# seulbinHwang/DiffusionDrive

Measured on AMD Instinct MI355X. Metric: scenes/s at batch 64, 2 denoise steps, 1/2/4/8 MI355X; waypoint L2 vs ref, higher is better.
Workload: dtype fp32 via f16x3 (each fp32 operand = hi+lo fp16, products ah*bh+ah*bl+al*bh, fp32 accumulate)

## Files before the change

diffusiondrive_amd/_lib.py:

```python
import ctypes
import os
import threading

HERE = os.path.dirname(os.path.abspath(__file__))
LIB_PATH = os.environ.get("DDMI_LIB", os.path.join(HERE, "libddmi.so"))

c_float_p = ctypes.POINTER(ctypes.c_float)
c_void_p = ctypes.c_void_p


class DDMIUnavailable(RuntimeError):
    """Raised when the native HIP library cannot be loaded."""


class DDMIError(RuntimeError):
    """Raised when a ddmi C-ABI call returns a non-zero status."""


class DDConfig(ctypes.Structure):
    _fields_ = [
        ("abi_version", ctypes.c_int), ("image_arch", ctypes.c_int), ("lidar_arch", ctypes.c_int),
        ("cam_h", ctypes.c_int), ("cam_w", ctypes.c_int), ("lidar_h", ctypes.c_int),
        ("lidar_w", ctypes.c_int), ("lidar_channels", ctypes.c_int), ("num_modes", ctypes.c_int),
        ("num_poses", ctypes.c_int), ("trunc_timestep", ctypes.c_int), ("step_span", ctypes.c_int),
    ]


class DDOutputs(ctypes.Structure):
    _fields_ = [
        ("trajectory", c_void_p), ("poses_reg", c_void_p), ("poses_cls", c_void_p),
        ("bev_semantic_map", c_void_p), ("agent_states", c_void_p), ("agent_labels", c_void_p),
    ]


class DDTrainOutputs(ctypes.Structure):
    _fields_ = [
        ("trajectory", c_void_p), ("poses_reg", c_void_p * 2), ("poses_cls", c_void_p * 2), ("loss", c_void_p),
        ("bev_semantic_map", c_void_p), ("agent_states", c_void_p), ("agent_labels", c_void_p),
    ]


class DDSampleOutputs(ctypes.Structure):
    _fields_ = [
        ("trajectory", c_void_p), ("poses_reg", c_void_p), ("poses_cls", c_void_p),
        ("best_trajectory", c_void_p), ("best_index", c_void_p),
        ("bev_semantic_map", c_void_p), ("agent_states", c_void_p), ("agent_labels", c_void_p),
    ]


class DDInputs(ctypes.Structure):
    _fields_ = [
        ("camera_f32", c_void_p), ("camera_u8", c_void_p), ("lidar_f32", c_void_p), ("lidar_u8", c_void_p),
        ("lidar_hist_max", ctypes.c_int), ("status", c_void_p), ("noise", c_void_p),
    ]


class DDSimParams(ctypes.Structure):
    _fields_ = [
        ("wheel_base", ctypes.c_double), ("dt", ctypes.c_double), ("tracking_horizon", ctypes.c_int),
        ("q_lon", ctypes.c_double), ("r_lon", ctypes.c_double), ("q_lat", ctypes.c_double * 3),
        ("r_lat", ctypes.c_double), ("jerk_penalty", ctypes.c_double), ("curvature_rate_penalty", ctypes.c_double),
        ("initial_curvature_penalty", ctypes.c_double), ("stopping_gain", ctypes.c_double),
        ("stopping_velocity", ctypes.c_double), ("max_steering_angle", ctypes.c_double),
        ("accel_time_constant", ctypes.c_double), ("steering_time_constant", ctypes.c_double),
    ]


class DDComfortParams(ctypes.Structure):
    _fields_ = [
        ("dt", ctypes.c_double), ("min_lon_accel", ctypes.c_double), ("max_lon_accel", ctypes.c_double),
        ("max_abs_lat_accel", ctypes.c_double), ("max_abs_mag_jerk", ctypes.c_double),
        ("max_abs_lon_jerk", ctypes.c_double), ("max_abs_yaw_accel", ctypes.c_double),
        ("max_abs_yaw_rate", ctypes.c_double),
    ]


class DDAreaParams(ctypes.Structure):
    _fields_ = [
        ("half_length", ctypes.c_double), ("half_width", ctypes.c_double), ("rear_axle_to_center", ctypes.c_double),
        ("dt", ctypes.c_double), ("driving_direction_horizon", ctypes.c_double),
        ("driving_direction_compliance_threshold", ctypes.c_double),
        ("driving_direction_violation_threshold", ctypes.c_double),
    ]


class DDDrivableMaps(ctypes.Structure):
    _fields_ = [
        ("verts", c_void_p), ("ring_off", c_void_p), ("poly_ring_off", c_void_p), ("poly_kind", c_void_p),
        ("scene_poly_off", c_void_p), ("num_polys", ctypes.c_int),
    ]


class DDOpView(ctypes.Structure):
    _fields_ = [("p", c_void_p), ("sn", ctypes.c_int64), ("sh", ctypes.c_int64), ("sw", ctypes.c_int64),
                ("sc", ctypes.c_int64)]


class DDOpConvDesc(ctypes.Structure):
    _fields_ = [
        ("in_", DDOpView), ("out", DDOpView), ("res", DDOpView),
        ("N", ctypes.c_int), ("H", ctypes.c_int), ("W", ctypes.c_int), ("Cin", ctypes.c_int),
        ("KH", ctypes.c_int), ("KW", ctypes.c_int), ("stride", ctypes.c_int), ("pad", ctypes.c_int),
        ("Cout", ctypes.c_int),
        ("wgt", c_void_p), ("ldb", ctypes.c_int64), ("k0", ctypes.c_int), ("bias", c_void_p),
        ("relu", ctypes.c_int), ("mode", ctypes.c_int), ("flags", c_void_p), ("route_rows", ctypes.c_int64),
        ("ln_out", c_void_p), ("ln_g", c_void_p), ("ln_b", c_void_p),
        ("pool_out", DDOpView), ("pool_p", ctypes.c_int), ("pool_add", DDOpView),
        ("fused_ln", ctypes.c_int), ("fused_pool", ctypes.c_int),
    ]


MAX_SAMPLES = 32

_SIGS = {
    "dd_default_config": (None, [ctypes.POINTER(DDConfig)]),
    "dd_create": (ctypes.c_int, [ctypes.POINTER(DDConfig), c_void_p, ctypes.c_size_t, ctypes.c_int,
                                 ctypes.POINTER(c_void_p)]),
    "dd_forward": (ctypes.c_int, [c_void_p, c_void_p, c_void_p, c_void_p, c_void_p, ctypes.c_int, ctypes.c_int,
                                  c_void_p, c_void_p, c_void_p, c_void_p]),
    "dd_forward_ex": (ctypes.c_int, [c_void_p, c_void_p, c_void_p, c_void_p, c_void_p, ctypes.c_int,
                                     ctypes.c_int, ctypes.POINTER(DDOutputs), c_void_p]),
    "dd_forward_samples": (ctypes.c_int, [c_void_p, c_void_p, c_void_p, c_void_p, c_void_p, ctypes.c_int,
                                          ctypes.c_int, ctypes.c_int, ctypes.POINTER(DDSampleOutputs), c_void_p]),
    "dd_forward_in": (ctypes.c_int, [c_void_p, ctypes.POINTER(DDInputs), ctypes.c_int, ctypes.c_int,
                                     ctypes.POINTER(DDOutputs), c_void_p]),
    "dd_forward_samples_in": (ctypes.c_int, [c_void_p, ctypes.POINTER(DDInputs), ctypes.c_int, ctypes.c_int,
                                             ctypes.c_int, ctypes.POINTER(DDSampleOutputs), c_void_p]),
    "dd_forward_train_in": (ctypes.c_int, [c_void_p, ctypes.POINTER(DDInputs), c_void_p, c_void_p, ctypes.c_int,
                                           ctypes.c_float, ctypes.c_float, c_void_p, c_void_p]),
    "dd_destroy": (ctypes.c_int, [c_void_p]),
    "dd_last_error": (ctypes.c_char_p, []),
    "dd_set_profiling": (ctypes.c_int, [c_void_p, ctypes.c_int]),
    "dd_reset_stats": (ctypes.c_int, [c_void_p]),
    "dd_kernel_stats": (ctypes.c_int, [c_void_p, ctypes.c_char_p, ctypes.POINTER(ctypes.c_double),
                                       ctypes.POINTER(ctypes.c_longlong), ctypes.POINTER(ctypes.c_double)]),
    "dd_kernel_bytes": (ctypes.c_int, [c_void_p, ctypes.c_char_p, ctypes.POINTER(ctypes.c_double)]),
    "dd_set_seed": (ctypes.c_int, [c_void_p, ctypes.c_ulonglong]),
    "dd_set_seed_at": (ctypes.c_int, [c_void_p, ctypes.c_ulonglong, ctypes.c_ulonglong]),
    "dd_set_graph": (ctypes.c_int, [c_void_p, ctypes.c_int]),
    "dd_set_streams": (ctypes.c_int, [c_void_p, ctypes.c_int]),
    "dd_get_streams": (ctypes.c_int, [c_void_p, ctypes.POINTER(ctypes.c_int)]),
    "dd_graph_info": (ctypes.c_int, [c_void_p, ctypes.POINTER(ctypes.c_int), ctypes.POINTER(ctypes.c_int),
                                     ctypes.POINTER(ctypes.c_int)]),
    "dd_graph_nodes": (ctypes.c_int, [c_void_p, ctypes.POINTER(ctypes.c_int), ctypes.POINTER(ctypes.c_int)]),
    "dd_forward_train": (ctypes.c_int, [c_void_p, c_void_p, c_void_p, c_void_p, c_void_p, c_void_p, c_void_p,
                                        ctypes.c_int, ctypes.c_float, ctypes.c_float, c_void_p, c_void_p]),
    "dd_bev_semantic_loss": (ctypes.c_int, [c_void_p, c_void_p, ctypes.c_int, ctypes.c_int, ctypes.c_int, ctypes.c_int,
                                            c_void_p, c_void_p, c_void_p]),
    "dd_bev_semantic_loss_work": (ctypes.c_size_t, [ctypes.c_int, ctypes.c_int, ctypes.c_int]),
    "dd_default_sim_params": (None, [ctypes.POINTER(DDSimParams)]),
    "dd_simulate_work": (ctypes.c_size_t, [ctypes.c_int]),
    "dd_simulate_proposals": (ctypes.c_int, [c_void_p, c_void_p, ctypes.c_int, ctypes.c_int,
                                             ctypes.POINTER(DDSimParams), c_void_p, c_void_p, c_void_p]),
    "dd_simulate": (ctypes.c_int, [c_void_p, ctypes.c_int, c_void_p, ctypes.c_int, ctypes.c_int,
                                   ctypes.POINTER(DDSimParams), c_void_p, c_void_p, c_void_p]),
    "dd_default_comfort_params": (None, [ctypes.POINTER(DDComfortParams)]),
    "dd_comfort": (ctypes.c_int, [c_void_p, ctypes.c_int, ctypes.POINTER(DDComfortParams), c_void_p, c_void_p,
                                  c_void_p]),
    "dd_default_area_params": (None, [ctypes.POINTER(DDAreaParams)]),
    "dd_ego_areas_work": (ctypes.c_size_t, [ctypes.c_int]),
    "dd_ego_areas": (ctypes.c_int, [c_void_p, ctypes.c_int, ctypes.c_int, ctypes.POINTER(DDDrivableMaps), ctypes.c_int,
                                    ctypes.POINTER(DDAreaParams), c_void_p, c_void_p, c_void_p, c_void_p, c_void_p,
                                    c_void_p]),
    "dd_set_gemm_mode": (ctypes.c_int, [c_void_p, ctypes.c_int]),
    "dd_set_schedule": (ctypes.c_int, [c_void_p, ctypes.c_int]),
    "dd_get_gemm_mode": (ctypes.c_int, [c_void_p, ctypes.POINTER(ctypes.c_int)]),
    "dd_numerics_flags": (ctypes.c_int, [c_void_p, ctypes.POINTER(ctypes.c_uint), ctypes.c_int]),
    "dd_tap": (ctypes.c_int, [c_void_p, ctypes.c_char_p, c_void_p, ctypes.c_size_t,
                              ctypes.POINTER(ctypes.c_size_t), c_void_p]),
    "dd_op_last_error": (ctypes.c_char_p, []),
    "dd_op_last_kernel": (ctypes.c_char_p, []),
    "dd_op_split_weights": (ctypes.c_int, [c_void_p, ctypes.c_int, ctypes.c_int, c_void_p, c_void_p, c_void_p, c_void_p,
                                           ctypes.POINTER(ctypes.c_int)]),
    "dd_op_pack_mk_weights": (ctypes.c_int, [c_void_p, ctypes.c_int, ctypes.c_int, c_void_p, c_void_p]),
    "dd_op_mk_linear": (ctypes.c_int, [c_void_p, ctypes.c_int, c_void_p, c_void_p, c_void_p, ctypes.c_int, c_void_p]),
    "dd_op_bevproj": (ctypes.c_int, [c_void_p, ctypes.c_int64, c_void_p, c_void_p, c_void_p, c_void_p, c_void_p, c_void_p,
                                     ctypes.c_int, ctypes.c_int, ctypes.c_int, ctypes.c_int, ctypes.c_int, c_void_p]),
    "dd_build_camera": (ctypes.c_int, [c_void_p, ctypes.c_int, ctypes.c_int, ctypes.c_int, c_void_p, ctypes.c_int,
                                       ctypes.c_int, c_void_p]),
    "dd_build_lidar": (ctypes.c_int, [c_void_p, c_void_p, ctypes.c_int, ctypes.c_int, c_void_p, ctypes.c_int,
                                      ctypes.c_float, ctypes.c_float, ctypes.c_int, ctypes.c_float, ctypes.c_float,
                                      ctypes.c_int, ctypes.c_longlong, c_void_p]),
    "dd_build_camera_u8": (ctypes.c_int, [c_void_p, ctypes.c_int, ctypes.c_int, ctypes.c_int, c_void_p, ctypes.c_int,
                                          ctypes.c_int, c_void_p]),
    "dd_build_lidar_u8": (ctypes.c_int, [c_void_p, c_void_p, ctypes.c_int, ctypes.c_int, c_void_p, ctypes.c_int,
                                         ctypes.c_float, ctypes.c_float, ctypes.c_int, ctypes.c_float, ctypes.c_float,
                                         ctypes.c_int, ctypes.c_longlong, c_void_p]),
    "dd_op_stem_pool_u8": (ctypes.c_int, [c_void_p, ctypes.c_int, ctypes.c_int, ctypes.c_int, ctypes.c_int,
                                          ctypes.c_int, c_void_p, c_void_p, c_void_p, c_void_p, ctypes.c_int, c_void_p,
                                          c_void_p]),
    "dd_op_conv2d": (ctypes.c_int, [c_void_p, ctypes.c_int, ctypes.c_int, ctypes.c_int, ctypes.c_int, c_void_p,
                                    c_void_p, c_void_p, c_void_p, ctypes.c_int, ctypes.c_int, ctypes.c_int,
                                    ctypes.c_int, ctypes.c_int, ctypes.c_int, c_void_p]),
    "dd_op_conv2d_x3": (ctypes.c_int, [c_void_p, ctypes.c_int, ctypes.c_int, ctypes.c_int, ctypes.c_int, c_void_p,
                                       c_void_p, c_void_p, c_void_p, ctypes.c_int, ctypes.c_int, ctypes.c_int,
                                       ctypes.c_int, ctypes.c_int, ctypes.c_int, ctypes.c_int, c_void_p, c_void_p]),
    "dd_op_stem_pool_x3": (ctypes.c_int, [c_void_p, ctypes.c_int, ctypes.c_int, ctypes.c_int, c_void_p, c_void_p,
                                          c_void_p, c_void_p, c_void_p]),
    "dd_op_stem_pool": (ctypes.c_int, [c_void_p, ctypes.c_int, ctypes.c_int, ctypes.c_int, c_void_p, c_void_p,
                                       c_void_p, ctypes.c_int, c_void_p, c_void_p]),
    "dd_op_stem_pool_nchw": (ctypes.c_int, [c_void_p, ctypes.c_int, ctypes.c_int, ctypes.c_int, ctypes.c_int, c_void_p,
                                            c_void_p, c_void_p, ctypes.c_int, c_void_p, c_void_p]),
    "dd_op_gemm": (ctypes.c_int, [c_void_p, ctypes.c_int, ctypes.c_int, c_void_p, c_void_p, c_void_p, c_void_p,
                                  ctypes.c_int, ctypes.c_int, c_void_p]),
    "dd_op_gemm_batched": (ctypes.c_int, [c_void_p, c_void_p, c_void_p, ctypes.c_int, ctypes.c_int, ctypes.c_int,
                                          ctypes.c_int, ctypes.c_int, c_void_p]),
    "dd_op_layernorm": (ctypes.c_int, [c_void_p, c_void_p, ctypes.c_int, c_void_p, c_void_p, c_void_p, c_void_p,
                                       c_void_p, ctypes.c_int, ctypes.c_int, c_void_p]),
    "dd_op_softmax_rows": (ctypes.c_int, [c_void_p, ctypes.c_int, ctypes.c_int, ctypes.c_float, c_void_p]),
    "dd_op_bilinear": (ctypes.c_int, [c_void_p, ctypes.c_int, ctypes.c_int, ctypes.c_int, ctypes.c_int, c_void_p,
                                      ctypes.c_int, ctypes.c_int, c_void_p]),
    "dd_op_bilinear_add": (ctypes.c_int, [c_void_p, ctypes.c_int, ctypes.c_int, ctypes.c_int, ctypes.c_int, c_void_p,
                                          ctypes.c_int, ctypes.c_int, c_void_p]),
    "dd_op_maxpool3x3s2": (ctypes.c_int, [c_void_p, ctypes.c_int, ctypes.c_int, ctypes.c_int, ctypes.c_int,
                                          c_void_p, c_void_p]),
    "dd_op_avgpool": (ctypes.c_int, [c_void_p, ctypes.c_int, ctypes.c_int, ctypes.c_int, ctypes.c_int,
                                     ctypes.c_int, ctypes.c_int, c_void_p, c_void_p]),
    "dd_op_bev_sample_attn": (ctypes.c_int, [c_void_p, c_void_p, c_void_p, c_void_p, ctypes.c_int, ctypes.c_int,
                                             ctypes.c_int, ctypes.c_int, ctypes.c_int, ctypes.c_int, c_void_p]),
    "dd_op_mha_small": (ctypes.c_int, [c_void_p, c_void_p, c_void_p, c_void_p, ctypes.c_int, ctypes.c_int,
                                       ctypes.c_int, ctypes.c_int, ctypes.c_int, c_void_p]),
    "dd_op_gpt_attention": (ctypes.c_int, [c_void_p, c_void_p, ctypes.c_int, ctypes.c_int, ctypes.c_int,
                                           ctypes.c_int, ctypes.c_int, c_void_p]),
    "dd_op_gpt_attention_rows": (ctypes.c_int, [c_void_p, c_void_p, ctypes.c_int, ctypes.c_int, ctypes.c_int,
                                                ctypes.c_int, ctypes.c_int, ctypes.c_int, ctypes.c_int, ctypes.c_int,
                                                c_void_p]),
    "dd_op_layernorm_groups": (ctypes.c_int, [c_void_p, c_void_p, c_void_p, c_void_p, ctypes.c_int, ctypes.c_int,
                                              ctypes.c_longlong, ctypes.c_int, c_void_p]),
    "dd_op_conv_desc_size": (ctypes.c_size_t, []),
    "dd_op_conv_view": (ctypes.c_int, [ctypes.POINTER(DDOpConvDesc), c_void_p]),
    "dd_op_layernorm_ld": (ctypes.c_int, [c_void_p, ctypes.c_int64, c_void_p, ctypes.c_int64, ctypes.c_int, c_void_p,
                                          c_void_p, c_void_p, c_void_p, ctypes.c_int, ctypes.c_int64, c_void_p,
                                          ctypes.c_int64, ctypes.c_int, ctypes.c_int, c_void_p]),
    "dd_op_bilinear_view": (ctypes.c_int, [ctypes.POINTER(DDOpView), ctypes.c_int, ctypes.c_int, ctypes.c_int,
                                           ctypes.c_int, ctypes.POINTER(DDOpView), ctypes.c_int, ctypes.c_int,
                                           ctypes.c_int, c_void_p]),
}

EXPORTED = tuple(_SIGS)

_lib = None
_lock = threading.Lock()


def load(path: str = None):
    global _lib
    with _lock:
        if _lib is not None and path is None:
            return _lib
        p = path or LIB_PATH
        if not os.path.exists(p):
            raise DDMIUnavailable(
                f"ddmi native library not found at {p}; build it with `python -m diffusiondrive_amd.build`")
        try:
            lib = ctypes.CDLL(p, mode=ctypes.RTLD_GLOBAL)
        except OSError as e:
            raise DDMIUnavailable(f"cannot load {p}: {e}") from e
        for name, (res, args) in _SIGS.items():
            fn = getattr(lib, name)
            fn.restype = res
            fn.argtypes = args
        if path is None:
            _lib = lib
        return lib


def check(rc: int, lib=None, op: bool = False):
    if rc != 0:
        lib = lib or load()
        msg = (lib.dd_op_last_error() if op else lib.dd_last_error()) or b""
        raise DDMIError(f"ddmi call failed (rc={rc}): {msg.decode(errors='replace')}")
    return rc
```

diffusiondrive_amd/csrc/common.h:

```cpp
#pragma once
#include <hip/hip_runtime.h>
#include <atomic>
#include <cstdint>
#include <stdexcept>
#include <string>

#define DD_HIP_CHECK(expr)                                                              \
  do {                                                                                   \
    hipError_t _e = (expr);                                                              \
    if (_e != hipSuccess)                                                                \
      throw std::runtime_error(std::string("HIP error ") + hipGetErrorString(_e) +      \
                               " at " __FILE__ ":" + std::to_string(__LINE__) + ": " #expr); \
  } while (0)

struct dd_sim_params;
struct dd_comfort_params;
struct dd_area_params;
struct dd_drivable_maps;

namespace ddmi {

inline void set_max_lds_once(std::atomic<uint64_t>& mask, const void* kernel, int bytes) {
  int dev = 0;
  DD_HIP_CHECK(hipGetDevice(&dev));
  const uint64_t bit = uint64_t(1) << (dev & 63);
  if (mask.load(std::memory_order_acquire) & bit) return;
  DD_HIP_CHECK(hipFuncSetAttribute(kernel, hipFuncAttributeMaxDynamicSharedMemorySize, bytes));
  mask.fetch_or(bit, std::memory_order_acq_rel);
}

struct View4 {
  float* p = nullptr;
  int64_t sn = 0, sh = 0, sw = 0, sc = 1;
};
inline View4 hwc(const float* p, int64_t sn, int W, int C) {
  return {const_cast<float*>(p), sn, (int64_t)W * C, C, 1};
}
inline View4 nhwc(const float* p, int H, int W, int C) { return hwc(p, (int64_t)H * W * C, W, C); }
inline View4 channels_from(View4 v, int64_t c0) {
  v.p += c0 * v.sc;
  return v;
}
inline View4 row_view(const float* p, int64_t gs, int64_t rs) { return {const_cast<float*>(p), gs, rs, 0, 1}; }

struct ConvArgs {
  const float* in = nullptr;
  int64_t in_sn = 0, in_sh = 0, in_sw = 0;
  int H = 1, W = 1, Cin = 0;
  const float* wgt = nullptr;
  int64_t ldb = 0;
  int b_kn = 0;
  const float* bias = nullptr;
  const float* res = nullptr;
  int64_t res_sn = 0, res_sh = 0, res_sw = 0;
  float* out = nullptr;
  int64_t out_sn = 0, out_sh = 0, out_sw = 0;
  int Nimg = 1, Ho = 1, Wo = 1, Cout = 0;
  int KH = 1, KW = 1, stride = 1, pad = 0;
  int relu = 0;
  float alpha = 1.0f;
  float* split_part = nullptr;
  int64_t split_cap = 0;
  int batch = 1, zdiv = 1;
  int64_t in_z1 = 0, in_z2 = 0, w_z1 = 0, w_z2 = 0, out_z1 = 0, out_z2 = 0, res_z1 = 0, res_z2 = 0;
  int64_t flops_K = -1;
  const uint16_t* wh = nullptr;
  const uint16_t* wl = nullptr;
  const float* wsinv = nullptr;
  int64_t ldh = 0;
  unsigned* flags = nullptr;
  int prec = 0;
  const int* rowmap = nullptr;
  int rowmap_nimg = 0;
  int rowmap_groups = 0;
  const int* rowcount = nullptr;
  int rowcap = 0;
  float* pool_out = nullptr;
  int pool_p = 0;
  int64_t pool_sn = 0, pool_sh = 0, pool_sw = 0;
  const float* pool_add = nullptr;
  int64_t pool_add_sh = 0, pool_add_sw = 0;
  float* ln_out = nullptr;
  const float* ln_g = nullptr;
  const float* ln_b = nullptr;
  int64_t route_rows = 0;
};
struct ConvGeom {
  int KH = 1, KW = 1, stride = 1, pad = 0, Cout = 0;
};
inline ConvArgs conv_args(View4 in, int N, int H, int W, int Cin, ConvGeom g, View4 out, int relu = 0,
                          View4 res = {}) {
  ConvArgs a;
  a.in = in.p;
  a.in_sn = in.sn;
  a.in_sh = in.sh;
  a.in_sw = in.sw;
  a.H = H;
  a.W = W;
  a.Cin = Cin;
  a.ldb = (int64_t)g.KH * g.KW * Cin;
  a.res = res.p;
  a.res_sn = res.sn;
  a.res_sh = res.sh;
  a.res_sw = res.sw;
  a.out = out.p;
  a.out_sn = out.sn;
  a.out_sh = out.sh;
  a.out_sw = out.sw;
  a.Nimg = N;
  a.Ho = (H + 2 * g.pad - g.KH) / g.stride + 1;
  a.Wo = (W + 2 * g.pad - g.KW) / g.stride + 1;
  a.Cout = g.Cout;
  a.KH = g.KH;
  a.KW = g.KW;
  a.stride = g.stride;
  a.pad = g.pad;
  a.relu = relu;
  return a;
}
inline ConvArgs gemm_args(View4 A, int G, int R, int K, int N, View4 C, int relu = 0, View4 res = {}) {
  return conv_args(A, G, R, 1, K, ConvGeom{1, 1, 1, 0, N}, C, relu, res);
}
inline void slice_k(ConvArgs& a, int k0, int64_t ldb) {
  a.wgt += k0;
  a.ldb = ldb;
  if (a.wh) a.wh += k0;
  if (a.wl) a.wl += k0;
}
inline void fold_ln(ConvArgs& a, float* y, const float* g, const float* b) {
  a.ln_out = y;
  a.ln_g = g;
  a.ln_b = b;
}
inline void pool_into(ConvArgs& a, int p, View4 out, View4 add) {
  a.pool_out = out.p;
  a.pool_p = p;
  a.pool_sn = out.sn;
  a.pool_sh = out.sh;
  a.pool_sw = out.sw;
  a.pool_add = add.p;
  a.pool_add_sh = add.sh;
  a.pool_add_sw = add.sw;
}
inline ConvArgs gathered_rows(ConvArgs a, const int* rowmap, int MR, int groups = 0, const int* counts = nullptr) {
  a.rowmap = rowmap;
  a.rowmap_nimg = a.Nimg;
  a.rowmap_groups = groups;
  if (counts) {
    a.rowcount = counts;
    a.rowcap = MR / groups;
  }
  a.Nimg = 1;
  a.Ho = MR;
  a.Wo = 1;
  return a;
}
constexpr unsigned DD_NUM_F16_OVERFLOW = 1u;
constexpr unsigned DD_NUM_SYNC_TIMEOUT = 2u;
constexpr unsigned DD_NUM_SYNC_STATE = 4u;
constexpr int kSplitMaxExp = 126;

#ifdef __HIPCC__
template <int BM, int NT>
__device__ inline void epi_row_table(const ConvArgs& a, int m0, int M, int tid, long long* tab,
                                     const int* rowidx = nullptr) {
  for (int r = tid; r < BM; r += NT) {
    const int m = rowidx ? rowidx[r] : m0 + r;
    long long oo = -1, ro = 0;
    if (m >= 0 && m < M) {
      const int ow = m % a.Wo, t2 = m / a.Wo;
      const int oh = t2 % a.Ho, n = t2 / a.Ho;
      oo = (long long)n * a.out_sn + (long long)oh * a.out_sh + (long long)ow * a.out_sw;
      ro = (long long)n * a.res_sn + (long long)oh * a.res_sh + (long long)ow * a.res_sw;
    }
    tab[2 * r] = oo;
    tab[2 * r + 1] = ro;
  }
}

__device__ inline void rowcount_prefix(const int* counts, int n, int* pre) {
  const int tid = threadIdx.x;
  if (tid < 64) {
    int c[4], s = 0;
#pragma unroll
    for (int j = 0; j < 4; ++j) {
      const int i = 4 * tid + j;
      c[j] = i < n ? counts[i] : 0;
      s += c[j];
    }
    int inc = s;
#pragma unroll
    for (int o = 1; o < 64; o <<= 1) {
      const int v = __shfl_up(inc, o, 64);
      if (tid >= o) inc += v;
    }
    int run = inc - s;
#pragma unroll
    for (int j = 0; j < 4; ++j) {
      const int i = 4 * tid + j;
      if (i <= n) pre[i] = run;
      run += c[j];
    }
    if (tid == 63 && n == 256) pre[256] = run;
  }
  __syncthreads();
}

__host__ __device__ inline bool epi_quads_ok(const ConvArgs& a) {
  auto al = [](const void* p) { return (reinterpret_cast<uintptr_t>(p) & 15) == 0; };
  auto st4 = [](int64_t s, int n) { return n == 1 || s % 4 == 0; };
  return a.Cout % 4 == 0 && al(a.out) && al(a.wsinv) && (!a.bias || al(a.bias)) && st4(a.out_sn, a.Nimg) &&
         st4(a.out_sh, a.Ho) && st4(a.out_sw, a.Wo) &&
         (!a.res || (al(a.res) && st4(a.res_sn, a.Nimg) && st4(a.res_sh, a.Ho) && st4(a.res_sw, a.Wo)));
}
template <int WM, int WN, int TM, int TN>
constexpr int epi_quads_lds() {
  return WM * 32 * WN * TN * 32 * 4 + WM * TM * 32 * 16;
}

template <int WM, int WN, int TM, int TN, typename Acc>
__device__ inline bool epi_quads(const ConvArgs& a, const Acc (&acc)[TM][TN], char* lds, int m0, int n0, int M,
                                 int tid, const int* rowidx = nullptr) {
  typedef float f4_t __attribute__((ext_vector_type(4)));
  constexpr int NT = 64 * WM * WN, BN = WN * TN * 32, QN = BN / 4, PR = WM * 32;
  constexpr int RPP = NT / QN, IT = PR / RPP;
  static_assert(NT % QN == 0 && PR % RPP == 0 && BN >= 64, "quad epilogue tiling");
  const int wave = tid >> 6, lane = tid & 63;
  const int wm = wave / WN, wn = wave % WN, li = lane & 31, hh = lane >> 5;
  float* ct = reinterpret_cast<float*>(lds);
  long long* tab = reinterpret_cast<long long*>(lds + PR * BN * 4);
  epi_row_table<WM * TM * 32, NT>(a, m0, M, tid, tab, rowidx);
  const int qn = tid % QN, nq = n0 + 4 * qn;
  const bool nv = nq < a.Cout;
  f4_t scl = {0.f, 0.f, 0.f, 0.f}, bia = {0.f, 0.f, 0.f, 0.f};
  if (nv) {
    scl = *reinterpret_cast<const f4_t*>(a.wsinv + nq) * a.alpha;
    if (a.bias) bia = *reinterpret_cast<const f4_t*>(a.bias + nq);
  }
  const bool ln = a.ln_out && BN == a.Cout && (QN == 16 || QN == 32 || QN == 64);
  f4_t lg = {0.f, 0.f, 0.f, 0.f}, lb = {0.f, 0.f, 0.f, 0.f};
  if (ln) {
    lg = *reinterpret_cast<const f4_t*>(a.ln_g + nq);
    lb = *reinterpret_cast<const f4_t*>(a.ln_b + nq);
  }
  bool bad = false;
#pragma unroll
  for (int i = 0; i < TM; ++i) {
    if (i) __syncthreads();
#pragma unroll
    for (int j = 0; j < TN; ++j)
#pragma unroll
      for (int r = 0; r < 16; ++r) {
        const int pr = wm * 32 + (r & 3) + 8 * (r >> 2) + 4 * hh;
        const int col = (wn * TN + j) * 32 + li;
        ct[pr * BN + ((((col >> 2) ^ (((pr >> 2) & 1) << 3))) << 2) + (col & 3)] = acc[i][j][r];
      }
    __syncthreads();
    f4_t rv[IT];
    long long oo[IT];
#pragma unroll
    for (int k = 0; k < IT; ++k) {
      const int pr = tid / QN + k * RPP;
      const int tr = ((pr >> 5) * TM + i) * 32 + (pr & 31);
      oo[k] = nv ? tab[2 * tr] : -1;
      rv[k] = (a.res && oo[k] >= 0) ? *reinterpret_cast<const f4_t*>(a.res + tab[2 * tr + 1] + nq)
                                    : (f4_t){0.f, 0.f, 0.f, 0.f};
    }
#pragma unroll
    for (int k = 0; k < IT; ++k) {
      if (oo[k] < 0) continue;
      const int pr = tid / QN + k * RPP;
      const f4_t c = *reinterpret_cast<const f4_t*>(ct + pr * BN + ((qn ^ (((pr >> 2) & 1) << 3)) << 2));
      bad |= !(__builtin_isfinite(c.x) && __builtin_isfinite(c.y) && __builtin_isfinite(c.z) &&
               __builtin_isfinite(c.w));
      f4_t v = c * scl + bia + rv[k];
      if (a.relu) {
        v.x = fmaxf(v.x, 0.f);
        v.y = fmaxf(v.y, 0.f);
        v.z = fmaxf(v.z, 0.f);
        v.w = fmaxf(v.w, 0.f);
      }
      __builtin_nontemporal_store(v, reinterpret_cast<f4_t*>(a.out + oo[k] + nq));
      if (ln) {
#pragma clang fp contract(off)
        float s = 0.f;
        s += (v.x + v.y) + (v.z + v.w);
#pragma unroll
        for (int o = QN / 2; o > 0; o >>= 1) s += __shfl_xor(s, o, 64);
        const float mean = s / (float)BN;
        const float dx = v.x - mean, dy = v.y - mean, dz = v.z - mean, dw = v.w - mean;
        float q = 0.f;
        q += (dx * dx + dy * dy) + (dz * dz + dw * dw);
#pragma unroll
        for (int o = QN / 2; o > 0; o >>= 1) q += __shfl_xor(q, o, 64);
        const float rstd = rsqrtf(q / (float)BN + 1e-5f);
        f4_t o4;
        o4.x = (v.x - mean) * rstd * lg.x + lb.x;
        o4.y = (v.y - mean) * rstd * lg.y + lb.y;
        o4.z = (v.z - mean) * rstd * lg.z + lb.z;
        o4.w = (v.w - mean) * rstd * lg.w + lb.w;
        *reinterpret_cast<f4_t*>(a.ln_out + oo[k] + nq) = o4;
      }
    }
  }
  return bad;
}
#endif
struct ConvRoute {
  const char* kernel = nullptr;
  const char* config = "";
  bool pooled = false;
  bool ln = false;
};
ConvRoute launch_conv_gemm(const ConvArgs& a, hipStream_t st);
ConvRoute launch_conv_x3(const ConvArgs& a, hipStream_t st);
ConvRoute launch_stem_pool(const ConvArgs& a, float* pool_out, int Hp, int Wp, hipStream_t st,
                           const void* const* src = nullptr, int src_c = 0, int u8 = 0, const float* lut = nullptr);
void launch_set_ptrs(const void** tab, const void* a, const void* b, hipStream_t st);
void launch_lidar_lut(float* lut, int hist_max, hipStream_t st);

struct VprojArgs {
  const float* map = nullptr;
  const uint16_t* wh = nullptr;
  const uint16_t* wl = nullptr;
  const float* wsinv = nullptr;
  int ldh = 0;
  const float* bias = nullptr;
  const int* rows = nullptr;
  const int* counts = nullptr;
  int B = 0, cap = 0;
  int nimg = 0;
  float* part = nullptr;
  float* out = nullptr;
  unsigned* flags = nullptr;
  int union_stage = 1;
  int umax = 1 << 30;
  unsigned* fb = nullptr;
  int fb_only = 0;
  int usplit = 1;
  unsigned* ucnt = nullptr;
};
bool vproj_supported(int C, int Cout, int H, int W);
size_t vproj_tiles(int B, int cap);
void launch_vproj(const VprojArgs& a, hipStream_t st);

void launch_nchw_to_nhwc(const float* in, float* out, int B, int C, int H, int W, int Cp, hipStream_t st);
void launch_u8_to_nhwc4(const uint8_t* in, float* out, int B, int C, int H, int W, int hwc, const float* lut,
                        hipStream_t st);
void launch_maxpool3x3s2(const float* in, float* out, int B, int H, int W, int C, int Ho, int Wo,
                         hipStream_t st);
void launch_avgpool(const float* in, int B, int H, int W, int C, int oh, int ow, View4 out,
                    const float* add, hipStream_t st);
void launch_bilinear(View4 in, int B, int Hi, int Wi, int C, View4 out, int Ho, int Wo, float ratio_h,
                     float ratio_w, int accumulate, hipStream_t st);
void launch_layernorm(const float* x, int64_t ldx, const float* res, int64_t ldres, int res_div,
                      const float* g, const float* b, const float* film_scale, const float* film_shift,
                      float* y, int64_t ldy, int rows, int C, hipStream_t st, int film_div = 0,
                      int64_t film_ld = 0, int group_rows = 0, int64_t group_stride = 0);
void launch_gpt_attention(const float* qkv, int B, int T, int C, int heads, float* y, int prec, hipStream_t st,
                          int q_first = 0, int q_count = -1, int nw_force = 0);
struct GptTailW {
  const uint16_t* wh = nullptr;
  const uint16_t* wl = nullptr;
  const float* sinv = nullptr;
  const float* bias = nullptr;
  int ldh = 0;
  float alpha = 1.0f;
};
struct GptTailArgs {
  const float* y = nullptr;
  float* x = nullptr;
  float* hb = nullptr;
  int M = 0, C = 0;
  GptTailW proj, up, down;
  const float *ln2_g = nullptr, *ln2_b = nullptr, *lnn_g = nullptr, *lnn_b = nullptr;
  unsigned* flags = nullptr;
};
bool gpt_tail_supported(int C);
void launch_gpt_tail(const GptTailArgs& a, hipStream_t st);
void launch_softmax_rows(float* x, int64_t ld, int rows, int L, float scale, hipStream_t st);
void launch_broadcast_rows(const float* src, int nsrc, float* dst, int rows, int C, hipStream_t st);
void launch_activation(const float* x, float* y, int64_t n, int act, hipStream_t st);
void launch_normal_philox(float* out, int64_t n, uint64_t seed, uint64_t first, hipStream_t st);

void launch_camera_feature(const uint8_t* cams, int B, int H, int W, float* out, int oh, int ow, hipStream_t st);
void launch_lidar_feature(const float* xyz, const int64_t* offs, int B, int C, float* out, int nb, float lo,
                          float hi, int ppm, float max_h, float split_h, int hist_max, int64_t max_points,
                          hipStream_t st);
void launch_camera_feature_u8(const uint8_t* cams, int B, int H, int W, uint8_t* out, int oh, int ow, hipStream_t st);
void launch_lidar_feature_u8(const float* xyz, const int64_t* offs, int B, int C, uint8_t* out, int nb, float lo,
                             float hi, int ppm, float max_h, float split_h, int hist_max, int64_t max_points,
                             hipStream_t st);

void launch_ddim_init(const float* anchor, const float* noise, float* img, int B, int QP, float sa,
                      float s1a, hipStream_t st);
void decoder_init_constants();
void launch_traj_embed(const float* img, float* pts, float* emb, int rows, int P, hipStream_t st);
void launch_timestep_embed(float t, float* out, int dim, hipStream_t st);
void launch_bev_sample_attn(const float* logits, const float* pts, const float* value, float* out,
                            int B, int Q, int P, int Hv, int Wv, int C, float inv_max_x,
                            float inv_max_y, hipStream_t st, int samples = 1);
void launch_bev_tap_rows(const float* pts, int* rows, int B, int Q, int P, int Hv, int Wv, float inv_max_x,
                         float inv_max_y, hipStream_t st, int samples = 1);
bool launch_bev_tap_dedup(const float* pts, int* rows, int* slots, int B, int Q, int P, int Hv, int Wv,
                          float inv_max_x, float inv_max_y, hipStream_t st, int samples = 1);
void launch_bev_sample_attn_gathered(const float* logits, const float* pts, const float* vrows, const int* slots,
                                     float* out, int B, int Q, int P, int Hv, int Wv, int C, float inv_max_x,
                                     float inv_max_y, hipStream_t st);
void launch_mha_small(const float* q, int64_t ldq, const float* k, const float* v, int64_t ldkv,
                      float* out, int64_t ldo, int B, int Lq, int Lk, int nh, int hd,
                      int64_t q_bstride, int64_t kv_bstride, int64_t o_bstride, hipStream_t st, int kv_div = 1);
void launch_reg_finalize(const float* r, const float* pts, float* reg, float* pts_next, int rows, int P,
                         hipStream_t st);
void launch_ddim_step(const float* reg, float* img, int rows, int P, float a_t, float a_prev,
                      hipStream_t st);
void launch_select_mode(const float* cls, const float* reg, float* traj, int* idx, int B, int Q, int P,
                        hipStream_t st);
void launch_select_best(const float* cls, const float* reg, float* traj, int* idx, int B, int N, int P,
                        hipStream_t st);
void launch_agent_post(float* states, int rows, hipStream_t st);

void launch_train_coeffs(const int* t, const float* ac, float* sa, float* s1a, int B, int tmax, hipStream_t st);
void launch_train_noisy(const float* anchor, const float* noise, const float* sa, const float* s1a, float* img, int B,
                        int QP, hipStream_t st);
void launch_timestep_embed_rows(const int* t, float* out, int B, int dim, hipStream_t st);
void launch_traj_loss_scene(const float* reg, const float* cls, const float* target, const float* anchor, float* part,
                            int B, int Q, int P, hipStream_t st);
void launch_traj_loss_reduce(const float* part, float* out, int B, int Q, int P, float cls_w, float reg_w,
                             hipStream_t st);
void launch_add2(float* o, hipStream_t st);
size_t bev_ce_partials(int B, int HW);
void launch_bev_ce(const float* logits, const uint8_t* target, float* part, float* out, int B, int C, int HW,
                   hipStream_t st);

size_t simulate_work_doubles(int N);
void launch_simulate(const float* traj, const double* proposals, const double* ego_states, int N, int per_group,
                     const dd_sim_params& p, double* work, double* out_states, hipStream_t st);

void launch_comfort(const double* states, int N, const dd_comfort_params& p, uint8_t* out_flags, double* out_signals,
                    hipStream_t st);

size_t ego_areas_work_doubles(int P);
void launch_ego_areas(const double* states, int N, int per_group, const dd_drivable_maps& maps, int G,
                      const dd_area_params& p, int horizon, double* work, uint8_t* out_areas, double* out_scores,
                      double* out_progress, double* out_coords, hipStream_t st);

}
```

diffusiondrive_amd/csrc/conv_x6.hip:

```cpp
#include <type_traits>

#include "common.h"


namespace ddmi {

namespace {

typedef _Float16 x6h8 __attribute__((ext_vector_type(8)));
typedef _Float16 x6h2 __attribute__((ext_vector_type(2)));
typedef float x6f2 __attribute__((ext_vector_type(2)));
typedef float x6f4 __attribute__((ext_vector_type(4)));
typedef float x6f16 __attribute__((ext_vector_type(16)));
typedef int x6i4 __attribute__((ext_vector_type(4)));
typedef __bf16 x6b8 __attribute__((ext_vector_type(8)));
typedef __bf16 x6b2 __attribute__((ext_vector_type(2)));

constexpr uint32_t kOOB6 = 0x80000000u;

__device__ inline x6i4 rsrc6(const void* p) {
  const uint64_t a = reinterpret_cast<uint64_t>(p);
  x6i4 r;
  r.x = (int)(uint32_t)a;
  r.y = (int)((uint32_t)(a >> 32) & 0xffffu);
  r.z = (int)kOOB6;
  r.w = 0x00020000;
  r.x = __builtin_amdgcn_readfirstlane(r.x);
  r.y = __builtin_amdgcn_readfirstlane(r.y);
  return r;
}

__device__ inline void dma6(x6i4 rsrc, uint32_t lds_wave, uint32_t voff) {
  asm volatile("s_mov_b32 m0, %0\n\tbuffer_load_dwordx4 %1, %2, 0 offen lds" ::"s"(lds_wave), "v"(voff), "s"(rsrc)
               : "memory");
}

__device__ inline x6f4 vload6(x6i4 rsrc, uint32_t voff) {
  x6f4 v;
  asm volatile("buffer_load_dwordx4 %0, %1, %2, 0 offen" : "=v"(v) : "v"(voff), "s"(rsrc) : "memory");
  return v;
}

template <int N>
__device__ inline void step_barrier() {
  static_assert(N >= 0 && N < 64, "vmcnt");
#ifdef DDMI_X6_NOBAR
  asm volatile("s_waitcnt vmcnt(%0) lgkmcnt(0)" ::"n"(N) : "memory");
#else
  asm volatile("s_waitcnt vmcnt(%0) lgkmcnt(0)\n\ts_barrier" ::"n"(N) : "memory");
#endif
}

template <int N>
__device__ inline void wait_vm() {
  static_assert(N >= 0 && N < 64, "vmcnt");
  asm volatile("s_waitcnt vmcnt(%0)" ::"n"(N) : "memory");
}

__device__ inline void split4(const x6f4 v, uint2& hi, uint2& lo) {
  const x6h2 h01 = __builtin_convertvector((x6f2){v.x, v.y}, x6h2);
  const x6h2 h23 = __builtin_convertvector((x6f2){v.z, v.w}, x6h2);
  const x6f2 f01 = __builtin_convertvector(h01, x6f2);
  const x6f2 f23 = __builtin_convertvector(h23, x6f2);
  const x6h2 l01 = __builtin_convertvector((x6f2){v.x - f01.x, v.y - f01.y}, x6h2);
  const x6h2 l23 = __builtin_convertvector((x6f2){v.z - f23.x, v.w - f23.y}, x6h2);
  hi = make_uint2(__builtin_bit_cast(uint32_t, h01), __builtin_bit_cast(uint32_t, h23));
  lo = make_uint2(__builtin_bit_cast(uint32_t, l01), __builtin_bit_cast(uint32_t, l23));
}

__device__ inline uint2 to_bf16x4(const x6f4 v) {
  const x6b2 b01 = __builtin_convertvector((x6f2){v.x, v.y}, x6b2);
  const x6b2 b23 = __builtin_convertvector((x6f2){v.z, v.w}, x6b2);
  return make_uint2(__builtin_bit_cast(uint32_t, b01), __builtin_bit_cast(uint32_t, b23));
}

constexpr bool halo_in_window(int t, int D, int TA, bool first) {
  for (int j = 1; j <= D; ++j) {
    const int u = t - j;
    if (first && u < 0) return false;
    if (((u % 9) + 9) % 9 == TA) return true;
  }
  return false;
}

}

#ifdef DDMI_X6_STAMPS
__device__ unsigned long long g_x6_st[8192 * 4];
extern "C" int dd_x6_stamps_read(unsigned long long* h, int n) {
  void* d = nullptr;
  if (hipGetSymbolAddress(&d, HIP_SYMBOL(g_x6_st)) != hipSuccess) return -1;
  if (hipMemcpy(h, d, (size_t)n * 8, hipMemcpyDeviceToHost) != hipSuccess) return -1;
  return hipMemset(d, 0, (size_t)n * 8) == hipSuccess ? 0 : -1;
}
#define X6_STAMP(k) x6st[k] = __builtin_amdgcn_s_memtime()
#else
#define X6_STAMP(k)
#endif

template <int TH, int TW, int BN, int WM, int WN, int D, int NSLOT, int SH, int PREC>
__global__ __launch_bounds__(64 * WM * WN, SH >= 2 ? SH + 1 : (SH ? (WM * WN == 8 ? 4 : 2) : 1)) void conv_x6_kernel(ConvArgs a, int tiles_x, int tiles_y, int n_sp,
                                                               int ntn, int nchunks) {
  constexpr int NW = WM * WN, NT = 64 * NW;
  constexpr int BM = TH * TW;
  constexpr int TM = BM / WM / 32;
  constexpr int TN = BN / WN / 32;
  static_assert(TM >= 1 && TN >= 1 && TM * WM * 32 == BM && TN * WN * 32 == BN, "wave tiling");
  static_assert(NSLOT >= D + 1 && D >= 1 && D <= 8, "ring");
  constexpr int P = TW + 2;
  constexpr int HP = (TH + 2) * P;
  constexpr int ABYTES = HP * 128;
  constexpr int BIMG = BN * 64;
  constexpr int BSLOT = 2 * BIMG;
  constexpr int BQ = BN / 16;
  constexpr int BPS = 2 * BQ / NW;
  static_assert(BPS >= 1 && (2 * BQ) % NW == 0 && BQ % BPS == 0, "B DMA split over the waves");
  constexpr int CH = PREC ? 64 : 32;
  constexpr int QP = CH / 4;
  constexpr int ALD = (HP * QP + NT - 1) / NT;
  constexpr int TA = 1;
  constexpr int NHB = SH ? 1 : 2;
  constexpr int B_OFF = NHB * ABYTES;
  constexpr int LDS_MAIN = NHB * ABYTES + NSLOT * BSLOT, LDS_EPI = BM * BN * 4;
  __shared__ __attribute__((aligned(1024))) char lds[LDS_MAIN > LDS_EPI ? LDS_MAIN : LDS_EPI];
  const uint32_t lds_u32 = (uint32_t)(uintptr_t)((__attribute__((address_space(3))) char*)lds);

  const int tid = threadIdx.x;
  const int lane = tid & 63;
  const int wave = __builtin_amdgcn_readfirstlane(tid >> 6);
#ifdef DDMI_X6_STAMPS
  unsigned long long x6st[4];
#endif
  X6_STAMP(0);

  const int nblk = n_sp * ntn;
  int tile = blockIdx.x;
  if (nblk >= 16) {
    const int q = nblk / 8, r = nblk % 8, x = tile % 8;
    tile = (x < r ? x * (q + 1) : r * (q + 1) + (x - r) * q) + tile / 8;
  }
  const int nt_idx = tile / n_sp;
  const int sp = tile - nt_idx * n_sp;
  const int txi = sp % tiles_x;
  const int t2 = sp / tiles_x;
  const int tyi = t2 % tiles_y;
  const int nimg = t2 / tiles_y;
  const int oy0 = tyi * TH, ox0 = txi * TW;
  const int n0 = nt_idx * BN;
  const int Cin = a.Cin;

  const x6i4 rin = rsrc6(a.in);

  constexpr bool HKEEP = NW == 8 && ALD <= 12 && !SH;
  auto hofs_of = [&](int i) {
    const int e = tid + NT * i;
    const int px = e / QP, q = e % QP;
    const int hy = px / P, hx = px - (px / P) * P;
    const int iy = oy0 - 1 + hy, ix = ox0 - 1 + hx;
    const bool in = px < HP && (unsigned)iy < (unsigned)a.H && (unsigned)ix < (unsigned)a.W;
    return in ? (int)(nimg * a.in_sn + iy * a.in_sh + ix * a.in_sw) + 4 * q : -1;
  };
  auto hwad_of = [&](int i) {
    const int e = tid + NT * i;
    const int px = e / QP, q = e % QP;
    const int q7 = q & 7, half = q >> 3;
    const int hx = px - (px / P) * P;
    return px < HP ? (px * 128 + ((((q7 >> 1) ^ (hx >> 1)) & 7) << 4) + ((q7 & 1) << 3)) ^ (half << 6) : -1;
  };
  int hofs[HKEEP ? ALD : 1], hwad[HKEEP ? ALD : 1];
  if constexpr (HKEEP) {
#pragma unroll
    for (int i = 0; i < ALD; ++i) {
      hofs[i] = hofs_of(i);
      hwad[i] = hwad_of(i);
    }
  }
  x6f4 hr[ALD];
  auto halo_issue = [&](int c) {
    const bool cv = c < nchunks;
    const int co = c * CH;
#pragma unroll
    for (int i = 0; i < ALD; ++i) {
      const int ho = HKEEP ? hofs[HKEEP ? i : 0] : hofs_of(i);
      hr[i] = vload6(rin, (cv && ho >= 0) ? (uint32_t)(ho + co) * 4u : kOOB6);
    }
  };
  auto halo_tie = [&]() {
#pragma unroll
    for (int i = 0; i < ALD; ++i) asm volatile("" : "+v"(hr[i]));
  };
  auto halo_store = [&](int buf) {
    char* base = lds + buf * ABYTES;
#pragma unroll
    for (int i = 0; i < ALD; ++i) {
      const int hw = HKEEP ? hwad[HKEEP ? i : 0] : hwad_of(i);
      if (hw < 0) continue;
      if constexpr (PREC == 1) {
        *reinterpret_cast<uint2*>(base + hw) = to_bf16x4(hr[i]);
      } else {
        uint2 hi, lo;
        split4(hr[i], hi, lo);
        *reinterpret_cast<uint2*>(base + hw) = hi;
        *reinterpret_cast<uint2*>(base + (hw ^ 64)) = lo;
      }
    }
  };

  uint32_t boff[BPS];
  bool bok[BPS];
  int brow[BPS];
#pragma unroll
  for (int j = 0; j < BPS; ++j) {
    const int qi = wave * BPS + j;
    const int rb = (qi % BQ) * 16;
    const int c = rb + (lane >> 2);
    const int ls = (lane & 3) ^ ((c >> 2) & 3);
    const int n = n0 + c;
    bok[j] = n < a.Cout;
    boff[j] = (uint32_t)(n * (int)a.ldh + ls * 8) * 2u;
    brow[j] = rb;
  }
  const bool bimg_lo = (wave * BPS) / BQ == 1;
  const x6i4 rwb = rsrc6((bimg_lo && !PREC) ? (const void*)a.wl : (const void*)a.wh);
  const uint32_t kb_lo = (PREC && bimg_lo) ? 64u : 0u;
  auto b_issue = [&](int slot, int tap, int c) {
    const bool cv = c < nchunks;
    const uint32_t kb = (uint32_t)(tap * Cin + c * CH) * 2u + kb_lo;
#pragma unroll
    for (int j = 0; j < BPS; ++j) {
      const uint32_t dst = lds_u32 + B_OFF + slot * BSLOT + (bimg_lo ? BIMG : 0) + brow[j] * 64;
      dma6(rwb, __builtin_amdgcn_readfirstlane(dst), (cv && bok[j]) ? boff[j] + kb : kOOB6);
    }
  };

  const int wm = wave / WN, wn = wave % WN;
  const int li = lane & 31, hh = lane >> 5;
  int aad[TM][3];
#pragma unroll
  for (int i = 0; i < TM; ++i) {
    const int m = (wm * TM + i) * 32 + li;
    const int y = m / TW, x = m % TW;
#pragma unroll
    for (int kw = 0; kw < 3; ++kw) aad[i][kw] = (y * P + x + kw) * 128 + (((hh ^ ((x + kw) >> 1)) & 7) << 4);
  }
  int bad_[TN];
#pragma unroll
  for (int j = 0; j < TN; ++j) {
    const int c = (wn * TN + j) * 32 + li;
    bad_[j] = c * 64 + (((hh ^ (c >> 2)) & 3) << 4);
  }

  x6f16 acc[TM][TN];
#pragma unroll
  for (int i = 0; i < TM; ++i)
#pragma unroll
    for (int j = 0; j < TN; ++j)
#pragma unroll
      for (int r = 0; r < 16; ++r) acc[i][j][r] = 0.f;

  constexpr bool PIPE = !(SH && NW == 8);
  struct Frag {
    x6h8 ah[TM], al[TM], bh[TN], bl[TN];
  };
  Frag F0, F1;
  auto load_frag = [&](Frag& F, int slot, int c, auto TAP, auto S2) {
    constexpr int t = decltype(TAP)::value, s2 = decltype(S2)::value;
    constexpr int kh = t / 3, kw = t % 3;
    const char* abuf = lds + (SH ? 0 : (c & 1)) * ABYTES + kh * P * 128;
    const char* bbuf = lds + B_OFF + slot * BSLOT;
#pragma unroll
    for (int j = 0; j < TN; ++j) {
      const int o = bad_[j] ^ (32 * s2);
      F.bh[j] = *reinterpret_cast<const x6h8*>(bbuf + o);
      F.bl[j] = *reinterpret_cast<const x6h8*>(bbuf + BIMG + o);
    }
#pragma unroll
    for (int i = 0; i < TM; ++i) {
      const int o = aad[i][kw] ^ (32 * s2);
      F.ah[i] = *reinterpret_cast<const x6h8*>(abuf + o);
      F.al[i] = *reinterpret_cast<const x6h8*>(abuf + (o ^ 64));
    }
  };
  auto mfma_frag = [&](const Frag& F) {
    if constexpr (PREC == 1) {
#pragma unroll
      for (int i = 0; i < TM; ++i)
#pragma unroll
        for (int j = 0; j < TN; ++j)
          acc[i][j] = __builtin_amdgcn_mfma_f32_32x32x16_bf16(__builtin_bit_cast(x6b8, F.ah[i]),
                                                             __builtin_bit_cast(x6b8, F.bh[j]), acc[i][j], 0, 0, 0);
#pragma unroll
      for (int i = 0; i < TM; ++i)
#pragma unroll
        for (int j = 0; j < TN; ++j)
          acc[i][j] = __builtin_amdgcn_mfma_f32_32x32x16_bf16(__builtin_bit_cast(x6b8, F.al[i]),
                                                             __builtin_bit_cast(x6b8, F.bl[j]), acc[i][j], 0, 0, 0);
      return;
    }
#pragma unroll
    for (int i = 0; i < TM; ++i)
#pragma unroll
      for (int j = 0; j < TN; ++j)
        acc[i][j] = __builtin_amdgcn_mfma_f32_32x32x16_f16(F.al[i], F.bh[j], acc[i][j], 0, 0, 0);
#pragma unroll
    for (int i = 0; i < TM; ++i)
#pragma unroll
      for (int j = 0; j < TN; ++j)
        acc[i][j] = __builtin_amdgcn_mfma_f32_32x32x16_f16(F.ah[i], F.bl[j], acc[i][j], 0, 0, 0);
#pragma unroll
    for (int i = 0; i < TM; ++i)
#pragma unroll
      for (int j = 0; j < TN; ++j)
        acc[i][j] = __builtin_amdgcn_mfma_f32_32x32x16_f16(F.ah[i], F.bh[j], acc[i][j], 0, 0, 0);
  };

  int slot = 0;
  auto open_step = [&](int c, auto TAP, auto FIRST) {
    constexpr int t = decltype(TAP)::value;
    constexpr bool first = decltype(FIRST)::value;
    constexpr int N = (D - 1) * BPS + (halo_in_window(t, D, TA, first) ? ALD : 0);
    step_barrier<N>();
    constexpr int tn = (t + D) % 9;
    int ns = slot + D;
    if (ns >= NSLOT) ns -= NSLOT;
    b_issue(ns, tn, t + D >= 9 ? c + 1 : c);
    if constexpr (t == TA) halo_issue(c + 1);
  };

  halo_issue(0);
#pragma unroll
  for (int u = 0; u < D; ++u) b_issue(u % NSLOT, u, 0);
  wait_vm<D * BPS>();
  halo_tie();
  halo_store(0);
  open_step(0, std::integral_constant<int, 0>(), std::true_type());
  if constexpr (PIPE) load_frag(F0, 0, 0, std::integral_constant<int, 0>(), std::integral_constant<int, 0>());

  auto step = [&](int c, auto TAP, auto FIRST) {
    constexpr int t = decltype(TAP)::value;
    constexpr bool first = decltype(FIRST)::value;
    if constexpr (!PIPE) {
      load_frag(F0, slot, c, TAP, std::integral_constant<int, 0>());
      mfma_frag(F0);
      load_frag(F0, slot, c, TAP, std::integral_constant<int, 1>());
      mfma_frag(F0);
      if constexpr (t == 8) {
        wait_vm<(8 - TA) * BPS>();
        halo_tie();
        asm volatile("s_waitcnt lgkmcnt(0)\n\ts_barrier" ::: "memory");
        halo_store(0);
      }
      if (++slot == NSLOT) slot = 0;
      open_step(t == 8 ? c + 1 : c, std::integral_constant<int, (t + 1) % 9>(),
                std::integral_constant<bool, first && t != 8>());
      return;
    }
    load_frag(F1, slot, c, TAP, std::integral_constant<int, 1>());
    __builtin_amdgcn_sched_barrier(0);
    mfma_frag(F0);
    if constexpr (t == 8) {
      wait_vm<(8 - TA) * BPS>();
      halo_tie();
      if constexpr (SH) {
        asm volatile("s_waitcnt lgkmcnt(0)\n\ts_barrier" ::: "memory");
        halo_store(0);
      } else {
        halo_store((c + 1) & 1);
      }
    }
    constexpr int t1 = (t + 1) % 9;
    const int c1 = t == 8 ? c + 1 : c;
    if (++slot == NSLOT) slot = 0;
    open_step(c1, std::integral_constant<int, t1>(), std::integral_constant<bool, first && t != 8>());
    load_frag(F0, slot, c1, std::integral_constant<int, t1>(), std::integral_constant<int, 0>());
    __builtin_amdgcn_sched_barrier(0);
    mfma_frag(F1);
    __builtin_amdgcn_sched_barrier(0);
  };
  auto chunk = [&](int c, auto FIRST) {
    step(c, std::integral_constant<int, 0>(), FIRST);
    step(c, std::integral_constant<int, 1>(), FIRST);
    step(c, std::integral_constant<int, 2>(), FIRST);
    step(c, std::integral_constant<int, 3>(), FIRST);
    step(c, std::integral_constant<int, 4>(), FIRST);
    step(c, std::integral_constant<int, 5>(), FIRST);
    step(c, std::integral_constant<int, 6>(), FIRST);
    step(c, std::integral_constant<int, 7>(), FIRST);
    step(c, std::integral_constant<int, 8>(), FIRST);
  };
  X6_STAMP(1);
  chunk(0, std::true_type());
  for (int c = 1; c < nchunks; ++c) chunk(c, std::false_type());
  step_barrier<0>();
  X6_STAMP(2);

  constexpr int QN = BN / 4;
  static_assert(NT % QN == 0, "epilogue quads");
  const int qn = tid % QN;
  const int nq = n0 + 4 * qn;
  const bool nv = nq < a.Cout;
  float* out = a.out + (int64_t)nimg * a.out_sn + nq;
  const float* res = a.res ? a.res + (int64_t)nimg * a.res_sn + nq : nullptr;
  const int osh = (int)a.out_sh, osw = (int)a.out_sw;
  const int rsh = (int)a.res_sh, rsw = (int)a.res_sw;
  constexpr int IT = BM / (NT / QN);
  constexpr bool EARLY = IT <= (NW == 8 && !SH ? 16 : 8);
  x6f4 rv[IT];
  int ooff[IT];
  auto load_res = [&]() {
#pragma unroll
    for (int k = 0; k < IT; ++k) {
      const int p = tid / QN + k * (NT / QN);
      const int oy = oy0 + p / TW, ox = ox0 + p % TW;
      const bool ok = nv && oy < a.Ho && ox < a.Wo;
      ooff[k] = ok ? oy * osh + ox * osw : -1;
      rv[k] = (res && ok) ? *reinterpret_cast<const x6f4*>(res + (oy * rsh + ox * rsw)) : (x6f4){0.f, 0.f, 0.f, 0.f};
    }
  };
  if constexpr (EARLY) load_res();
  x6f4 scl = {0.f, 0.f, 0.f, 0.f}, bia = {0.f, 0.f, 0.f, 0.f};
  if (nv) {
    scl = *reinterpret_cast<const x6f4*>(a.wsinv + nq) * a.alpha;
    if (a.bias) bia = *reinterpret_cast<const x6f4*>(a.bias + nq);
  }
  float* ct = reinterpret_cast<float*>(lds);
#pragma unroll
  for (int i = 0; i < TM; ++i)
#pragma unroll
    for (int j = 0; j < TN; ++j)
#pragma unroll
      for (int r = 0; r < 16; ++r) {
        const int m = (wm * TM + i) * 32 + (r & 3) + 8 * (r >> 2) + 4 * hh;
        ct[m * BN + (wn * TN + j) * 32 + li] = acc[i][j][r];
      }
  __syncthreads();
  if constexpr (!EARLY) load_res();
  bool bad = false;
#pragma unroll
  for (int k = 0; k < IT; ++k) {
    if (ooff[k] < 0) continue;
    const int p = tid / QN + k * (NT / QN);
    const x6f4 acc_v = *reinterpret_cast<const x6f4*>(ct + p * BN + 4 * qn);
    bad |= !(__builtin_isfinite(acc_v.x) && __builtin_isfinite(acc_v.y) && __builtin_isfinite(acc_v.z) &&
             __builtin_isfinite(acc_v.w));
    x6f4 v = acc_v * scl + bia + rv[k];
    if (a.relu) {
      v.x = fmaxf(v.x, 0.f);
      v.y = fmaxf(v.y, 0.f);
      v.z = fmaxf(v.z, 0.f);
      v.w = fmaxf(v.w, 0.f);
    }
    __builtin_nontemporal_store(v, reinterpret_cast<x6f4*>(out + ooff[k]));
    if (a.pool_out) *reinterpret_cast<x6f4*>(ct + p * BN + 4 * qn) = v;
  }
  if (a.pool_out) {
    __syncthreads();
    const int P = a.pool_p, WX = TW / P, NWIN = (TH / P) * WX;
    const float inv = 1.0f / (float)(P * P);
    for (int w = tid; w < NWIN * QN; w += NT) {
      const int win = w / QN, q = w - win * QN;
      const int nc = n0 + 4 * q;
      if (nc >= a.Cout) continue;
      const int wy = win / WX, wx = win - wy * WX;
      x6f4 sum = {0.f, 0.f, 0.f, 0.f};
      for (int dy = 0; dy < P; ++dy)
        for (int dx = 0; dx < P; ++dx)
          sum += *reinterpret_cast<const x6f4*>(ct + ((wy * P + dy) * TW + wx * P + dx) * BN + 4 * q);
      x6f4 v = sum * inv;
      const int py = oy0 / P + wy, px = ox0 / P + wx;
      if (a.pool_add) v += *reinterpret_cast<const x6f4*>(a.pool_add + py * a.pool_add_sh + px * a.pool_add_sw + nc);
      *reinterpret_cast<x6f4*>(a.pool_out + nimg * a.pool_sn + py * a.pool_sh + px * a.pool_sw + nc) = v;
    }
  }
  if (bad && a.flags) atomicOr(a.flags, (unsigned)DD_NUM_F16_OVERFLOW);
#ifdef DDMI_X6_STAMPS
  __syncthreads();
  X6_STAMP(3);
  if (tid == 0 && blockIdx.x < 8192)
    for (int k = 0; k < 4; ++k) g_x6_st[blockIdx.x * 4 + k] = x6st[k];
#endif
}

template <int TH, int TW, int BN, int WM, int WN, int D, int NSLOT, int SH, int PREC>
static void launch_x6_one(const ConvArgs& a_in, hipStream_t st, ConvRoute& r) {
  ConvArgs a = a_in;
  auto al16 = [](const void* p) { return (reinterpret_cast<uintptr_t>(p) & 15) == 0; };
  const bool pool = a.pool_out && a.pool_p >= 1 && TH % a.pool_p == 0 && TW % a.pool_p == 0 && a.Ho % TH == 0 &&
                    a.Wo % TW == 0 && al16(a.pool_out) && a.pool_sn % 4 == 0 && a.pool_sh % 4 == 0 &&
                    a.pool_sw % 4 == 0 && (!a.pool_add || (al16(a.pool_add) && a.pool_add_sh % 4 == 0 &&
                                                           a.pool_add_sw % 4 == 0));
  if (!pool) a.pool_out = nullptr;
  r.pooled = pool;
  const int tiles_x = (a.Wo + TW - 1) / TW, tiles_y = (a.Ho + TH - 1) / TH;
  const int n_sp = a.Nimg * tiles_x * tiles_y;
  const int ntn = (a.Cout + BN - 1) / BN;
  static const std::string name = "conv_x6<" + std::to_string(TH) + "," + std::to_string(TW) + "," +
                                  std::to_string(BN) + "," + std::to_string(WM) + "," + std::to_string(WN) +
                                  (PREC ? ",bf16>" : ">");
  r.config = name.c_str();
  hipLaunchKernelGGL((conv_x6_kernel<TH, TW, BN, WM, WN, D, NSLOT, SH, PREC>), dim3(n_sp * ntn), dim3(64 * WM * WN), 0,
                     st, a, tiles_x, tiles_y, n_sp, ntn, a.Cin / (PREC ? 64 : 32));
  DD_HIP_CHECK(hipGetLastError());
}
template <int TH, int TW, int BN, int WM, int WN, int D, int NSLOT, int SH>
static void launch_x6_cfg(const ConvArgs& a, hipStream_t st, ConvRoute& r) {
  if constexpr (SH == 0) {
    if (a.prec == 1) {
      launch_x6_one<TH, TW, BN, WM, WN, D, NSLOT, SH, 1>(a, st, r);
      return;
    }
  } else {
    if (a.prec == 1) throw std::runtime_error("conv_x6: bf16 takes the 8-wave configurations");
  }
  launch_x6_one<TH, TW, BN, WM, WN, D, NSLOT, SH, 0>(a, st, r);
}

bool launch_conv_x6(const ConvArgs& a, hipStream_t st, ConvRoute& r) {
  if ((a.prec != 0 && a.prec != 1) || a.KH != 3 || a.KW != 3 || a.stride != 1 || a.pad != 1 ||
      a.Cin % (a.prec ? 64 : 32) != 0 || a.batch != 1 || a.b_kn)
    return false;
  if (a.Ho != a.H || a.Wo != a.W || a.Ho < 8) return false;
  auto al16 = [](const void* p) { return (reinterpret_cast<uintptr_t>(p) & 15) == 0; };
  if (a.Cout % 4 || a.out_sw % 4 || a.out_sh % 4 || a.out_sn % 4 || !al16(a.out) || !al16(a.wsinv) ||
      (a.bias && !al16(a.bias)))
    return false;
  if (a.res && (a.res_sw % 4 || a.res_sh % 4 || a.res_sn % 4 || !al16(a.res))) return false;
  if ((int64_t)a.Nimg * a.in_sn >= (int64_t(1) << 29) || (int64_t)a.Cout * a.ldh >= (int64_t(1) << 30)) return false;
  if (a.Ho == 8 && a.Wo == 8 && a.Cout % 128 == 0) {
    if ((int64_t)a.Nimg * (a.Cout / 128) < 128) return false;
    launch_x6_cfg<8, 8, 128, 2, 4, 3, 4, 0>(a, st, r);
    return true;
  }
  const bool wide = a.Ho < 16;
  if (wide && a.Wo < 32) return false;
  const int64_t n_sp = (int64_t)a.Nimg * (wide ? ((a.Ho + 7) / 8) * ((a.Wo + 31) / 32)
                                               : ((a.Ho + 15) / 16) * ((a.Wo + 15) / 16));
  const bool bn128 = a.Cout > 64 && n_sp * ((a.Cout + 127) / 128) >= 256;
  const bool sh4 = a.prec == 0 && a.Cin <= 64;
  const bool b128 = bn128;
#define X6(TH, TW, BN, WM, WN, D, NS, SH) launch_x6_cfg<TH, TW, BN, WM, WN, D, NS, SH>(a, st, r)
  {
    const int64_t wgs = b128 ? n_sp * ((a.Cout + 127) / 128) : n_sp * ((a.Cout + 63) / 64);
    const char* se = getenv("DDMI_X6_SMALL");
    const int sm = se ? atoi(se) : 1;
    if (sm == 2 || (wgs < 128 && sm != 0)) {
      X6(8, 8, 64, 2, 2, 2, 3, 0);
      return true;
    }
  }
  if (wide) {
    if (b128) {
      X6(8, 32, 128, 4, 2, 3, 4, 0);
    } else {
      if (sh4) X6(8, 32, 64, 4, 1, 2, 3, 1); else X6(8, 32, 64, 4, 2, 2, 3, 0);
    }
  } else {
    if (b128) {
      X6(16, 16, 128, 4, 2, 3, 4, 0);
    } else {
      if (sh4) X6(16, 16, 64, 4, 1, 2, 3, 1); else X6(16, 16, 64, 4, 2, 2, 3, 0);
    }
  }
#undef X6
  return true;
}

}
```

diffusiondrive_amd/csrc/ops_abi.cpp:

```cpp
#include <cmath>
#include <cstring>
#include <string>

#include "../../include/ddmi.h"
#include "common.h"
#include "decoder_mk.h"
#include "weights.h"
#include <vector>

namespace {
thread_local std::string g_op_err;
thread_local const char* g_op_kernel = "";
void ran(const ddmi::ConvRoute& r) {
  if (*r.config) g_op_kernel = r.config;
}

template <class F>
int op_guard(F&& f) {
  try {
    f();
    return DD_OK;
  } catch (const std::invalid_argument& e) {
    g_op_err = e.what();
    return DD_ERR_INVALID;
  } catch (const std::exception& e) {
    g_op_err = e.what();
    return DD_ERR_RUNTIME;
  }
}
hipStream_t S(void* s) { return static_cast<hipStream_t>(s); }
}

using namespace ddmi;

extern "C" {

const char* dd_op_last_error(void) { return g_op_err.c_str(); }

const char* dd_op_last_kernel(void) { return g_op_kernel; }

int dd_op_split_weights(const float* w, int rows, int K, uint16_t* hi, uint16_t* lo, uint16_t* b16, float* sinv,
                        int* ldh_out) {
  return op_guard([&] {
    if (!w || rows < 1 || K < 1) throw std::invalid_argument("dd_op_split_weights: null pointer or bad shape");
    Arena ar;
    const SplitW x = prep_split(ar, w, rows, K);
    const size_t bytes = (size_t)rows * x.ldh * sizeof(uint16_t);
    if (hi) std::memcpy(hi, ar.host(x.hi), bytes);
    if (lo) std::memcpy(lo, ar.host(x.lo), bytes);
    if (b16) std::memcpy(b16, ar.host(x.b16), bytes);
    if (sinv) std::memcpy(sinv, ar.host(x.sinv), (size_t)rows * sizeof(float));
    if (ldh_out) *ldh_out = x.ldh;
  });
}

int dd_op_pack_mk_weights(const float* w, int nout, int nin, uint16_t* packed, float* sinv) {
  return op_guard([&] {
    if (!w || nout < 1 || nin < 1 || nin % 16 || nout % 32)
      throw std::invalid_argument("dd_op_pack_mk_weights: null pointer, nin % 16 or nout % 32");
    std::vector<_Float16> pk;
    std::vector<float> si;
    pack_mk_weights(w, nout, nin, pk, si);
    if (packed) std::memcpy(packed, pk.data(), pk.size() * sizeof(_Float16));
    if (sinv) std::memcpy(sinv, si.data(), si.size() * sizeof(float));
  });
}

int dd_op_mk_linear(const float* A, int K, const float* wgt, const float* bias, float* out, int N, void* stream) {
  return op_guard([&] {
    std::vector<float> hw((size_t)N * K);
    DD_HIP_CHECK(hipStreamSynchronize(S(stream)));
    DD_HIP_CHECK(hipMemcpy(hw.data(), wgt, hw.size() * sizeof(float), hipMemcpyDeviceToHost));
    std::vector<_Float16> pk;
    std::vector<float> sinv;
    pack_mk_weights(hw.data(), N, K, pk, sinv);
    Arena ar;
    const size_t wo = ar.add(reinterpret_cast<const float*>(pk.data()), pk.size() / 2);
    const size_t so = ar.add(sinv);
    ar.upload();
    MkLin m;
    m.w = reinterpret_cast<const uint4*>(ar.ptr(wo));
    m.s = ar.ptr(so);
    m.b = bias;
    m.nks = K / 16;
    launch_mk_linear_test(A, K, m, N, out, S(stream));
    DD_HIP_CHECK(hipStreamSynchronize(S(stream)));
  });
}

int dd_op_bevproj(const float* p3, int64_t p3_ld, const float* kvp, const float* wgt, const float* bias,
                  const float* ln_g, const float* ln_b, float* out, int B, int H, int W, int Hk, int Wk, void* stream) {
  return op_guard([&] {
    if (!bevproj_supported(256, 64, H, W, Hk, Wk)) throw std::invalid_argument("dd_op_bevproj: unsupported shape");
    std::vector<float> hw((size_t)256 * 64);
    DD_HIP_CHECK(hipStreamSynchronize(S(stream)));
    DD_HIP_CHECK(hipMemcpy(hw.data(), wgt, hw.size() * sizeof(float), hipMemcpyDeviceToHost));
    std::vector<_Float16> pk;
    std::vector<float> sinv;
    pack_mk_weights(hw.data(), 256, 64, pk, sinv);
    Arena ar;
    const size_t wo = ar.add(reinterpret_cast<const float*>(pk.data()), pk.size() / 2);
    const size_t so = ar.add(sinv);
    ar.upload();
    BevProjArgs a;
    a.p3 = p3;
    a.p3_ld = p3_ld;
    a.kvp = kvp;
    a.w = reinterpret_cast<const uint4*>(ar.ptr(wo));
    a.s = ar.ptr(so);
    a.bias = bias;
    a.g = ln_g;
    a.beta = ln_b;
    a.out = out;
    a.B = B;
    a.H = H;
    a.W = W;
    a.Hk = Hk;
    a.Wk = Wk;
    launch_bevproj(a, S(stream));
    DD_HIP_CHECK(hipStreamSynchronize(S(stream)));
  });
}

static ConvArgs conv2d_args(const float* in, int B, int H, int W, int Cin, const float* wgt, const float* bias,
                            const float* res, float* out, int Cout, int KH, int KW, int stride, int pad, int relu) {
  const int Ho = (H + 2 * pad - KH) / stride + 1, Wo = (W + 2 * pad - KW) / stride + 1;
  ConvArgs a = conv_args(nhwc(in, H, W, Cin), B, H, W, Cin, ConvGeom{KH, KW, stride, pad, Cout},
                         nhwc(out, Ho, Wo, Cout), relu, nhwc(res, Ho, Wo, Cout));
  a.wgt = wgt;
  a.bias = bias;
  return a;
}
static void attach_split(ConvArgs& a, const Arena& ar, const SplitW& x, int prec, unsigned* flags) {
  a.prec = prec;
  a.wh = reinterpret_cast<const uint16_t*>(ar.ptr(prec ? x.b16 : x.hi));
  a.wl = reinterpret_cast<const uint16_t*>(ar.ptr(x.lo));
  a.wsinv = ar.ptr(x.sinv);
  a.ldh = x.ldh;
  a.flags = flags;
}

int dd_op_conv2d(const float* in, int B, int H, int W, int Cin, const float* wgt, const float* bias, const float* res,
                 float* out, int Cout, int KH, int KW, int stride, int pad, int relu, void* stream) {
  return op_guard([&] {
    ran(launch_conv_gemm(conv2d_args(in, B, H, W, Cin, wgt, bias, res, out, Cout, KH, KW, stride, pad, relu),
                         S(stream)));
  });
}

int dd_op_conv2d_x3(const float* in, int B, int H, int W, int Cin, const float* wgt, const float* bias,
                    const float* res, float* out, int Cout, int KH, int KW, int stride, int pad, int relu, int prec,
                    unsigned* flags, void* stream) {
  return op_guard([&] {
    const int K = KH * KW * Cin;
    std::vector<float> hw((size_t)Cout * K);
    DD_HIP_CHECK(hipStreamSynchronize(S(stream)));
    DD_HIP_CHECK(hipMemcpy(hw.data(), wgt, hw.size() * sizeof(float), hipMemcpyDeviceToHost));
    Arena ar;
    const SplitW x = prep_split(ar, hw.data(), Cout, K);
    ar.upload();
    ConvArgs a = conv2d_args(in, B, H, W, Cin, wgt, bias, res, out, Cout, KH, KW, stride, pad, relu);
    if (prec != 0 && prec != 1) throw std::invalid_argument("prec must be 0 (f16x3) or 1 (bf16)");
    attach_split(a, ar, x, prec, flags);
    const int64_t mo = (int64_t)B * a.Ho * a.Wo * Cout;
    float* part = nullptr;
    if (prec == 0 && mo <= (1 << 20)) {
      DD_HIP_CHECK(hipMalloc(&part, (size_t)(8 * mo) * sizeof(float)));
      a.split_part = part;
      a.split_cap = 8 * mo;
    }
    ran(launch_conv_gemm(a, S(stream)));
    const hipError_t e = hipStreamSynchronize(S(stream));
    if (part) DD_HIP_CHECK(hipFree(part));
    DD_HIP_CHECK(e);
  });
}

static int dd_op_stem_pool_impl(const void* in, int src_c, int B, int H, int W, const float* wgt, const float* bias,
                                float* out, int prec, unsigned* flags, void* stream, int u8 = 0,
                                const float* lut = nullptr);

int dd_op_stem_pool_u8(const uint8_t* in, int layout, int B, int C, int H, int W, const float* lut, const float* wgt,
                       const float* bias, float* out, int prec, unsigned* flags, void* stream) {
  if (!in || !lut || (layout != 0 && layout != 1) || C < 1 || C > 3 || (layout == 0 && C != 3))
    return op_guard([&] {
      throw std::invalid_argument("stem_pool_u8: layout 0 (HWC, C = 3) or 1 (planar, C = 1..3), in and lut non-null");
    });
  return dd_op_stem_pool_impl(in, C, B, H, W, wgt, bias, out, prec, flags, stream, layout == 0 ? 1 : 2, lut);
}

int dd_op_stem_pool_x3(const float* in, int B, int H, int W, const float* wgt, const float* bias, float* out,
                       unsigned* flags, void* stream) {
  return dd_op_stem_pool(in, B, H, W, wgt, bias, out, 0, flags, stream);
}

int dd_op_stem_pool_nchw(const float* in, int B, int C, int H, int W, const float* wgt, const float* bias, float* out,
                         int prec, unsigned* flags, void* stream) {
  if (C < 1 || C > 3) return op_guard([&] { throw std::invalid_argument("stem_pool_nchw: C must be 1..3"); });
  return dd_op_stem_pool_impl(in, C, B, H, W, wgt, bias, out, prec, flags, stream);
}

int dd_op_stem_pool(const float* in, int B, int H, int W, const float* wgt, const float* bias, float* out, int prec,
                    unsigned* flags, void* stream) {
  return dd_op_stem_pool_impl(in, 0, B, H, W, wgt, bias, out, prec, flags, stream);
}

static int dd_op_stem_pool_impl(const void* in, int src_c, int B, int H, int W, const float* wgt, const float* bias,
                                float* out, int prec, unsigned* flags, void* stream, int u8, const float* lut) {
  return op_guard([&] {
    if (prec != 0 && prec != 1) throw std::invalid_argument("stem_pool: prec must be 0 (f16x3) or 1 (bf16)");
    const int Cin = 4, Cout = 64, K = 7 * 7 * Cin;
    std::vector<float> hw((size_t)Cout * K);
    DD_HIP_CHECK(hipStreamSynchronize(S(stream)));
    DD_HIP_CHECK(hipMemcpy(hw.data(), wgt, hw.size() * sizeof(float), hipMemcpyDeviceToHost));
    Arena ar;
    const SplitW x = prep_split(ar, hw.data(), Cout, K);
    ar.upload();
    ConvArgs a = conv_args(nhwc(u8 ? nullptr : static_cast<const float*>(in), H, W, Cin), B, H, W, Cin,
                           ConvGeom{7, 7, 2, 3, Cout}, View4{}, true);
    a.wgt = wgt;
    a.bias = bias;
    attach_split(a, ar, x, prec, flags);
    const int hp = (a.Ho + 2 - 3) / 2 + 1, wp = (a.Wo + 2 - 3) / 2 + 1;
    const void** word = nullptr;
    if (src_c) {
      DD_HIP_CHECK(hipMalloc(reinterpret_cast<void**>(&word), sizeof(const void*)));
      DD_HIP_CHECK(hipMemcpy(word, &in, sizeof(const void*), hipMemcpyHostToDevice));
    }
    bool ok = false;
    try {
      const ConvRoute r = launch_stem_pool(a, out, hp, wp, S(stream), src_c ? word : nullptr, src_c, u8, lut);
      ran(r);
      ok = r.kernel != nullptr;
      DD_HIP_CHECK(hipStreamSynchronize(S(stream)));
    } catch (...) {
      if (word) (void)hipFree(word);
      throw;
    }
    if (word) DD_HIP_CHECK(hipFree(word));
    if (!ok) throw std::invalid_argument("stem_pool: shape not supported");
  });
}

int dd_build_camera(const uint8_t* cams, int B, int src_h, int src_w, float* out, int out_h, int out_w,
                    void* stream) {
  return op_guard([&] {
    if (!cams || !out) throw std::invalid_argument("null pointer");
    launch_camera_feature(cams, B, src_h, src_w, out, out_h, out_w, S(stream));
  });
}

int dd_build_lidar(const float* xyz, const int64_t* offsets, int B, int channels, float* out, int resolution,
                   float range_lo, float range_hi, int pixels_per_meter, float max_height, float split_height,
                   int hist_max, long long max_points, void* stream) {
  return op_guard([&] {
    if (!offsets || !out || (!xyz && max_points > 0)) throw std::invalid_argument("null pointer");
    launch_lidar_feature(xyz, offsets, B, channels, out, resolution, range_lo, range_hi, pixels_per_meter,
                         max_height, split_height, hist_max, max_points, S(stream));
  });
}

int dd_build_camera_u8(const uint8_t* cams, int B, int src_h, int src_w, uint8_t* out, int out_h, int out_w,
                       void* stream) {
  return op_guard([&] {
    if (!cams || !out) throw std::invalid_argument("null pointer");
    launch_camera_feature_u8(cams, B, src_h, src_w, out, out_h, out_w, S(stream));
  });
}

int dd_build_lidar_u8(const float* xyz, const int64_t* offsets, int B, int channels, uint8_t* out, int resolution,
                      float range_lo, float range_hi, int pixels_per_meter, float max_height, float split_height,
                      int hist_max, long long max_points, void* stream) {
  return op_guard([&] {
    if (!offsets || !out || (!xyz && max_points > 0)) throw std::invalid_argument("null pointer");
    launch_lidar_feature_u8(xyz, offsets, B, channels, out, resolution, range_lo, range_hi, pixels_per_meter,
                            max_height, split_height, hist_max, max_points, S(stream));
  });
}

int dd_op_gemm(const float* A, int M, int K, const float* W, const float* bias, const float* res, float* C, int N,
               int relu, void* stream) {
  return op_guard([&] {
    ConvArgs a = gemm_args(row_view(A, K, K), M, 1, K, N, row_view(C, N, N), relu, row_view(res, N, N));
    a.wgt = W;
    a.bias = bias;
    ran(launch_conv_gemm(a, S(stream)));
  });
}

int dd_op_gemm_batched(const float* A, const float* Bm, float* C, int batch, int M, int N, int K, int kn,
                       void* stream) {
  return op_guard([&] {
    ConvArgs a = gemm_args(row_view(A, K, K), M, 1, K, N, row_view(C, N, N));
    a.wgt = Bm;
    a.ldb = kn ? N : K;
    a.b_kn = kn;
    a.batch = batch;
    a.zdiv = 1;
    a.in_z1 = (int64_t)M * K;
    a.w_z1 = (int64_t)K * N;
    a.out_z1 = (int64_t)M * N;
    ran(launch_conv_gemm(a, S(stream)));
  });
}

int dd_op_layernorm(const float* x, const float* res, int res_div, const float* g, const float* b,
                    const float* film_scale, const float* film_shift, float* y, int rows, int C, void* stream) {
  return op_guard([&] {
    launch_layernorm(x, C, res, C, res_div, g, b, film_scale, film_shift, y, C, rows, C, S(stream));
  });
}

int dd_bev_semantic_loss(const float* logits, const unsigned char* target, int B, int C, int H, int W, float* work,
                         float* loss, void* stream) {
  return op_guard([&] {
    if (!logits || !target || !work || !loss || B < 1 || C < 1 || C > 255 || H < 1 || W < 1)
      throw std::invalid_argument("dd_bev_semantic_loss: null pointer or bad shape");
    launch_bev_ce(logits, target, work, loss, B, C, H * W, S(stream));
  });
}

size_t dd_bev_semantic_loss_work(int B, int H, int W) { return bev_ce_partials(B, H * W); }

int dd_op_softmax_rows(float* x, int rows, int L, float scale, void* stream) {
  return op_guard([&] { launch_softmax_rows(x, L, rows, L, scale, S(stream)); });
}

int dd_op_bilinear(const float* in, int B, int Hi, int Wi, int C, float* out, int Ho, int Wo, void* stream) {
  return op_guard([&] {
    View4 a{const_cast<float*>(in), (int64_t)Hi * Wi * C, (int64_t)Wi * C, C, 1};
    View4 o{out, (int64_t)Ho * Wo * C, (int64_t)Wo * C, C, 1};
    launch_bilinear(a, B, Hi, Wi, C, o, Ho, Wo, (float)Hi / (float)Ho, (float)Wi / (float)Wo, 0, S(stream));
  });
}

int dd_op_bilinear_add(const float* in, int B, int Hi, int Wi, int C, float* out, int Ho, int Wo, void* stream) {
  return op_guard([&] {
    View4 a{const_cast<float*>(in), (int64_t)Hi * Wi * C, (int64_t)Wi * C, C, 1};
    View4 o{out, (int64_t)Ho * Wo * C, (int64_t)Wo * C, C, 1};
    launch_bilinear(a, B, Hi, Wi, C, o, Ho, Wo, (float)Hi / (float)Ho, (float)Wi / (float)Wo, 1, S(stream));
  });
}

int dd_op_maxpool3x3s2(const float* in, int B, int H, int W, int C, float* out, void* stream) {
  return op_guard([&] {
    const int Ho = (H + 2 - 3) / 2 + 1, Wo = (W + 2 - 3) / 2 + 1;
    launch_maxpool3x3s2(in, out, B, H, W, C, Ho, Wo, S(stream));
  });
}

int dd_op_avgpool(const float* in, int B, int H, int W, int C, int oh, int ow, float* out, void* stream) {
  return op_guard([&] {
    View4 o{out, (int64_t)oh * ow * C, (int64_t)ow * C, C, 1};
    launch_avgpool(in, B, H, W, C, oh, ow, o, nullptr, S(stream));
  });
}

int dd_op_bev_sample_attn(const float* logits, const float* pts, const float* value, float* out, int B, int Q, int P,
                          int Hv, int Wv, int C, void* stream) {
  return op_guard([&] {
    launch_bev_sample_attn(logits, pts, value, out, B, Q, P, Hv, Wv, C, 1.0f / 32.0f, 1.0f / 32.0f, S(stream));
  });
}

int dd_op_mha_small(const float* q, const float* k, const float* v, float* out, int B, int Lq, int Lk, int nh, int hd,
                    void* stream) {
  return op_guard([&] {
    const int d = nh * hd;
    launch_mha_small(q, d, k, v, d, out, d, B, Lq, Lk, nh, hd, (int64_t)Lq * d, (int64_t)Lk * d, (int64_t)Lq * d,
                     S(stream));
  });
}

int dd_op_gpt_attention(const float* qkv, float* y, int B, int T, int C, int heads, int prec, void* stream) {
  return op_guard([&] { launch_gpt_attention(qkv, B, T, C, heads, y, prec, S(stream)); });
}

int dd_op_gpt_attention_rows(const float* qkv, float* y, int B, int T, int C, int heads, int prec, int q_first,
                             int q_count, int waves, void* stream) {
  return op_guard([&] {
    if (q_count < 1) throw std::invalid_argument("dd_op_gpt_attention_rows: q_count < 1");
    launch_gpt_attention(qkv, B, T, C, heads, y, prec, S(stream), q_first, q_count, waves);
  });
}

int dd_op_layernorm_groups(const float* x, const float* g, const float* b, float* y, int groups, int group_rows,
                           long long group_stride, int C, void* stream) {
  return op_guard([&] {
    if (groups < 1 || group_rows < 1 || group_stride < (long long)group_rows * C)
      throw std::invalid_argument("dd_op_layernorm_groups: groups, group_rows >= 1 and non-overlapping groups");
    launch_layernorm(x, C, nullptr, 0, 1, g, b, nullptr, nullptr, y, C, groups * group_rows, C, S(stream), 0, 0,
                     group_rows, group_stride);
  });
}

size_t dd_op_conv_desc_size(void) { return sizeof(dd_op_conv_desc); }

static View4 view_of(const dd_op_view& v) { return {v.p, v.sn, v.sh, v.sw, v.sc}; }

int dd_op_conv_view(dd_op_conv_desc* d, void* stream) {
  return op_guard([&] {
    if (!d) throw std::invalid_argument("dd_op_conv_view: null descriptor");
    d->fused_ln = d->fused_pool = 0;
    if (!d->in.p || !d->out.p || !d->wgt) throw std::invalid_argument("dd_op_conv_view: null in, out or wgt");
    if (d->mode < 0 || d->mode > 2) throw std::invalid_argument("dd_op_conv_view: mode must be 0, 1 or 2");
    if (d->N < 1 || d->H < 1 || d->W < 1 || d->Cin < 1 || d->Cout < 1 || d->KH < 1 || d->KW < 1 || d->stride < 1 ||
        d->pad < 0)
      throw std::invalid_argument("dd_op_conv_view: bad geometry");
    for (const dd_op_view* v : {&d->in, &d->out, &d->res, &d->pool_out, &d->pool_add})
      if (v->p && v->sc != 1) throw std::invalid_argument("dd_op_conv_view: the operands' channel stride is 1");
    const int64_t K = (int64_t)d->KH * d->KW * d->Cin;
    const bool sliced = d->k0 != 0 || d->ldb != K;
    if (sliced && (d->KH != 1 || d->KW != 1 || d->k0 < 0 || d->k0 % 8 || d->Cin % 8 || d->k0 + K > d->ldb))
      throw std::invalid_argument("dd_op_conv_view: a K slice needs a 1 x 1 geometry, k0 % 8 == 0, Cin % 8 == 0 and "
                                  "k0 + Cin <= ldb");
    const ConvGeom g{d->KH, d->KW, d->stride, d->pad, d->Cout};
    const bool rows = d->KH == 1 && d->KW == 1 && d->stride == 1 && d->pad == 0 && d->W == 1;
    ConvArgs a = rows ? gemm_args(view_of(d->in), d->N, d->H, d->Cin, d->Cout, view_of(d->out), d->relu,
                                  view_of(d->res))
                      : conv_args(view_of(d->in), d->N, d->H, d->W, d->Cin, g, view_of(d->out), d->relu,
                                  view_of(d->res));
    a.wgt = d->wgt;
    a.bias = d->bias;
    a.route_rows = d->route_rows;
    Arena ar;
    DD_HIP_CHECK(hipStreamSynchronize(S(stream)));
    if (d->mode) {
      std::vector<float> hw((size_t)d->Cout * d->ldb);
      DD_HIP_CHECK(hipMemcpy(hw.data(), d->wgt, hw.size() * sizeof(float), hipMemcpyDeviceToHost));
      const SplitW x = prep_split(ar, hw.data(), d->Cout, (int)d->ldb);
      ar.upload();
      attach_split(a, ar, x, d->mode - 1, d->flags);
    }
    if (sliced) slice_k(a, d->k0, d->ldb);
    if (d->ln_out) fold_ln(a, d->ln_out, d->ln_g, d->ln_b);
    if (d->pool_out.p) pool_into(a, d->pool_p, view_of(d->pool_out), view_of(d->pool_add));
    const int64_t mo = (int64_t)a.Nimg * a.Ho * a.Wo * a.Cout;
    float* part = nullptr;
    if (d->mode == 1 && mo <= (1 << 20)) {
      DD_HIP_CHECK(hipMalloc(&part, (size_t)(8 * mo) * sizeof(float)));
      a.split_part = part;
      a.split_cap = 8 * mo;
    }
    hipError_t e = hipSuccess;
    try {
      const ConvRoute r = launch_conv_gemm(a, S(stream));
      ran(r);
      d->fused_ln = r.ln;
      d->fused_pool = r.pooled;
      e = hipStreamSynchronize(S(stream));
    } catch (...) {
      if (part) (void)hipFree(part);
      throw;
    }
    if (part) DD_HIP_CHECK(hipFree(part));
    DD_HIP_CHECK(e);
  });
}

int dd_op_layernorm_ld(const float* x, int64_t ldx, const float* res, int64_t ldres, int res_div, const float* g,
                       const float* b, const float* film_scale, const float* film_shift, int film_div,
                       int64_t film_ld, float* y, int64_t ldy, int rows, int C, void* stream) {
  return op_guard([&] {
    if (!x || !y || !g || !b || rows < 0 || C < 1 || ldx < C || ldy < C)
      throw std::invalid_argument("dd_op_layernorm_ld: null pointer or a leading dimension below C");
    launch_layernorm(x, ldx, res, ldres, res_div, g, b, film_scale, film_shift, y, ldy, rows, C, S(stream), film_div,
                     film_ld);
  });
}

int dd_op_bilinear_view(const dd_op_view* in, int B, int Hi, int Wi, int C, const dd_op_view* out, int Ho, int Wo,
                        int accumulate, void* stream) {
  return op_guard([&] {
    if (!in || !out || !in->p || !out->p || B < 1 || Hi < 1 || Wi < 1 || C < 1 || Ho < 1 || Wo < 1)
      throw std::invalid_argument("dd_op_bilinear_view: null view or bad shape");
    launch_bilinear(view_of(*in), B, Hi, Wi, C, view_of(*out), Ho, Wo, (float)Hi / (float)Ho, (float)Wi / (float)Wo,
                    accumulate, S(stream));
  });
}

}
```

diffusiondrive_amd/csrc/runtime.cpp:

```cpp
#include <cmath>
#include <cstdio>
#include <cstdlib>
#include <cstring>
#include <map>
#include <memory>
#include <mutex>
#include <set>
#include <type_traits>
#include <vector>

#ifdef DDMI_SEGV_TRACE
#define DD_TRACE(...) (fprintf(stderr, "[ddmi-trace] " __VA_ARGS__), fputc('\n', stderr), fflush(stderr))
#else
#define DD_TRACE(...) ((void)0)
#endif
#include "../../include/ddmi.h"
#include "common.h"
#include "decoder_mk.h"
#include "weights.h"

namespace ddmi {

struct Block {
  bool bottleneck = false;
// ... 746 lines not shown
      ia.rows = rows_of(0, 0);
      ia.slots = slots_of(0, 0);
      ia.counts = counts_of(0, 0);
      ia.sa = vanilla ? 0.0f : std::sqrt(a8);
      ia.s1a = vanilla ? 1.0f : std::sqrt(1.0f - a8);
      if (c.train) {
        ia.sa_b = bufs.at("train_sa").first;
        ia.s1a_b = bufs.at("train_s1a").first;
      }
      ia.B = B;
      ia.samples = S;
      launch("decoder", 0, [&] { launch_decoder_mk_init(ia, st); });
      launch("misc", 0, [&] {
        launch_mk_prefetch(W(mk_w_begin), (mk_w_end - mk_w_begin) * sizeof(float), st);
      });
    }
    const MkLayer layers[2] = {mk_layer(0), mk_layer(1)};
    MkAnchor anc;
    anc.pa0 = mk(m_pa0);
    anc.pa3 = mk(m_pa3);
    anc.pa2g = W(pa2.g);
    anc.pa2b = W(pa2.b);
    float* reg_last = nullptr;
    float* cls_last = nullptr;
    for (int si = 0; si < steps; ++si) {
      for (int l = 0; l < 2; ++l) {
        const std::string sf = sfx(si, l);
        float* vrows = buf("value_rows" + sf, (size_t)MR * d);
        gathered_value(l, rows_of(si, l), counts_of(si, l), vrows, cross, B, B / S, HB, WB, MR,
                       tf_pending ? tf_scenes : 0);
        if (tf_pending) {
          join();
          tf_pending = false;
        }
        MkArgs m;
        m.L = layers[l];
        m.A = anc;
        m.layer = l;
        m.B = B;
        m.samples = S;
        m.imgx = imgx;
        m.tfe = tfe;
        m.pts = l == 0 ? pts : pts2;
        m.pts_next = l == 0 ? pts2 : nullptr;
        m.vrows = vrows;
        m.slots = slots_of(si, l);
        m.akv = akv[l];
        m.ego = egos[l];
        if (c.train) {
          m.film = bufs.at("train_film_l" + std::to_string(l)).first;
          m.film_stride = 2 * d;
        } else {
          m.film = buf("film_s" + std::to_string(si) + "l" + std::to_string(l), 2 * d);
        }
        m.gs_out = buf("gs" + sf, (size_t)R * d);
        m.reg_out = buf("reg" + sf, (size_t)R * P * 3);
        m.cls_out = buf("cls" + sf, R);
        if (l == 0) {
          m.next_rows = rows_of(si, 1);
          m.next_slots = slots_of(si, 1);
          m.next_counts = counts_of(si, 1);
        } else if (si + 1 < steps) {
          m.next_rows = rows_of(si + 1, 0);
          m.next_slots = slots_of(si + 1, 0);
          m.next_counts = counts_of(si + 1, 0);
          const int k = roll[si];
          const float a_t = ac[k], a_p = (k - ratio >= 0) ? ac[k - ratio] : 1.0f;
          m.ddim = 1;
          m.sa_t = std::sqrt(a_t);
          m.sb_t = std::sqrt(1.0f - a_t);
          m.sa_p = std::sqrt(a_p);
          m.sdir = std::sqrt(1.0f - a_p);
        } else {
          m.traj = traj;
          m.mode_idx = idx;
        }
        m.flags = num_flags;
        m.dim_t = W(dim_t_off);
        m.groups = mk_stamps ? 1 : (mk_groups_env ? mk_groups_env : (B * 4 <= 64 ? 4 : (B * 2 <= 64 ? 2 : 1)));
        if (m.groups > 1) {
          m.scene_cnt = reinterpret_cast<unsigned*>(buf_zeroed("mk_scene_cnt", (size_t)B));
          m.next_pts = buf("mk_next_pts", (size_t)R * P * 2);
          m.cls_x = buf("mk_cls_x", (size_t)B * 32);
        }
        if (mk_stamps) m.stamps = reinterpret_cast<unsigned long long*>(buf("mk_stamps" + sf, (size_t)B * 80));
        double kn = 7.0 * d * d + 2.0 * d * 1024 + (double)d * (P + 1 + 3 * P);
        if (l == 0) kn += 512.0 * d + (double)d * d;
        launch("decoder", 2.0 * R * kn, [&] { launch_decoder_mk(m, st); }, nullptr, -1.0, groups_note(m.groups));
        reg_last = m.reg_out;
        cls_last = m.cls_out;
      }
    }
    join();
    alias("poses_reg", reg_last);
    alias("poses_cls", cls_last);
    train_loss_partials(c, B);
  }

  const float* W(size_t off) const { return ar.ptr(off); }

  int num_cus() {
    if (!cu_count) {
      int dev = 0;
      DD_HIP_CHECK(hipGetDevice(&dev));
      DD_HIP_CHECK(hipDeviceGetAttribute(&cu_count, hipDeviceAttributeMultiprocessorCount, dev));
    }
    return cu_count;
  }
  int cu_count = 0;

  float* buf_zeroed(const std::string& name, size_t n) {
    const uint64_t g = generation;
    float* p = buf(name, n);
    if (generation != g) DD_HIP_CHECK(hipMemsetAsync(p, 0, std::max<size_t>(n, 4) * sizeof(float), st));
    return p;
  }

  float* buf(const std::string& name, size_t n) {
    auto it = bufs.find(name);
    if (it != bufs.end() && it->second.second >= n) return it->second.first;
    if (it != bufs.end()) {
      DD_HIP_CHECK(hipFree(it->second.first));
      bufs.erase(it);
    }
    float* p = nullptr;
    DD_HIP_CHECK(hipMalloc(&p, std::max<size_t>(n, 4) * sizeof(float)));
    bufs[name] = {p, n};
    ++generation;
    return p;
  }

  hipEvent_t fj_event() {
    if (fj_next == fj_ev.size()) {
      hipEvent_t e;
      DD_HIP_CHECK(hipEventCreateWithFlags(&e, hipEventDisableTiming));
      fj_ev.push_back(e);
    }
    return fj_ev[fj_next++];
  }
  bool sides() const { return use_side && !profiling; }

  bool seg_cap = false;
  int seg_s = 0;
  hipStream_t st_cap = nullptr;
  Program* seg_prog = nullptr;
  void seg_begin(int s) {
    seg_s = s;
    DD_HIP_CHECK(hipStreamBeginCapture(st_cap, hipStreamCaptureModeThreadLocal));
  }
  void seg_end() {
    hipGraph_t g = nullptr;
    DD_HIP_CHECK(hipStreamEndCapture(st_cap, &g));
    size_t n = 0, roots = 0;
    hipError_t e = hipGraphGetNodes(g, nullptr, &n);
    if (e == hipSuccess) e = hipGraphGetRootNodes(g, nullptr, &roots);
    if (e == hipSuccess && n > 0) {
      if (roots > 1) ++seg_prog->branched;
      std::vector<hipGraphNode_t> nodes(n);
      e = hipGraphGetNodes(g, nodes.data(), &n);
      for (size_t i = 0; e == hipSuccess && i < n; ++i) {
        hipGraphNodeType ty;
        e = hipGraphNodeGetType(nodes[i], &ty);
        if (e == hipSuccess) ++(ty == hipGraphNodeTypeKernel ? seg_prog->kernel_nodes : seg_prog->other_nodes);
      }
    }
    if (e == hipSuccess && n > 0) {
      hipGraphExec_t ex = nullptr;
      e = hipGraphInstantiate(&ex, g, nullptr, nullptr, 0);
      if (e == hipSuccess) {
        seg_prog->ops.push_back({0, seg_s, ex, -1});
        ++seg_prog->segments;
      }
    }
    (void)hipGraphDestroy(g);
    DD_HIP_CHECK(e);
  }
  void seg_event(int from, int to) {
    const int e = (int)fj_next;
    (void)fj_event();
    seg_prog->ops.push_back({1, from, nullptr, e});
    seg_prog->ops.push_back({2, to, nullptr, e});
  }
  void fork() {
    if (!sides()) return;
    if (seg_cap) {
      seg_end();
      seg_event(0, 1);
      seg_begin(0);
      return;
    }
    hipEvent_t e = fj_event();
    DD_HIP_CHECK(hipEventRecord(e, st_main));
    DD_HIP_CHECK(hipStreamWaitEvent(st_side, e, 0));
  }
  void join() {
    if (!sides()) return;
    if (seg_cap) {
      seg_end();
      seg_event(1, 0);
      seg_begin(0);
      return;
    }
    hipEvent_t e = fj_event();
    DD_HIP_CHECK(hipEventRecord(e, st_side));
    DD_HIP_CHECK(hipStreamWaitEvent(st_main, e, 0));
  }
  bool in_side = false;
  template <class F>
  void side(F&& f) {
    struct SideFlag {
      bool& b;
      explicit SideFlag(bool& x) : b(x) { b = true; }
      ~SideFlag() { b = false; }
    } flag(in_side);
    if (seg_cap) {
      seg_end();
      seg_begin(1);
      f();
      seg_end();
      seg_begin(0);
      return;
    }
    st = sides() ? st_side : st_main;
    try {
      f();
    } catch (...) {
      st = st_main;
      throw;
    }
    st = st_main;
  }

  void capture_program(const Call& c, Program& p) {
    seg_prog = &p;
    st_cap = st;
    seg_cap = sides();
    try {
      seg_begin(0);
      forward_body(c);
      seg_end();
    } catch (...) {
      hipStreamCaptureStatus cs = hipStreamCaptureStatusNone;
      if (hipStreamIsCapturing(st_cap, &cs) == hipSuccess && cs != hipStreamCaptureStatusNone) {
        hipGraph_t dummy = nullptr;
        if (hipStreamEndCapture(st_cap, &dummy) == hipSuccess && dummy) (void)hipGraphDestroy(dummy);
      }
      (void)hipGetLastError();
      seg_cap = false;
      seg_prog = nullptr;
      destroy_program(p);
      throw;
    }
    seg_cap = false;
    seg_prog = nullptr;
  }
  void run_program(const Program& p) {
    const hipStream_t ss[2] = {st_main, st_side};
    for (const SegOp& op : p.ops) {
      if (op.kind == 0)
        DD_HIP_CHECK(hipGraphLaunch(op.ex, ss[op.s]));
      else if (op.kind == 1)
        DD_HIP_CHECK(hipEventRecord(fj_ev[op.ev], ss[op.s]));
      else
        DD_HIP_CHECK(hipStreamWaitEvent(ss[op.s], fj_ev[op.ev], 0));
    }
  }

  static const char* groups_note(int g) { return g == 4 ? "groups=4" : (g == 2 ? "groups=2" : "groups=1"); }

  template <class F>
  ConvRoute launch(const char* name, double flops, F&& f, const ConvArgs* shape = nullptr, double bytes = -1.0,
                   const char* note = nullptr) {
    ConvRoute route;
    auto run = [&] {
      if constexpr (std::is_void_v<decltype(f())>) f();
      else route = f();
    };
    if (!profiling) {
      run();
      return route;
    }
    hipEvent_t a, b;
    if (ev_pool.size() >= 2) {
      a = ev_pool.back();
      ev_pool.pop_back();
      b = ev_pool.back();
      ev_pool.pop_back();
    } else {
      DD_HIP_CHECK(hipEventCreate(&a));
      DD_HIP_CHECK(hipEventCreate(&b));
    }
    DD_HIP_CHECK(hipEventRecord(a, st));
    run();
    DD_HIP_CHECK(hipEventRecord(b, st));
    if (force_class) name = force_class;
    else if (shape) name = route.kernel;
    std::string detail;
    if (shape) {
      const ConvArgs& c = *shape;
      detail = "M=" + std::to_string((int64_t)c.Nimg * c.Ho * c.Wo) + " N=" + std::to_string(c.Cout) +
               " K=" + std::to_string(c.KH * c.KW * c.Cin) + " k=" + std::to_string(c.KH) + " s=" +
               std::to_string(c.stride) + " z=" + std::to_string(c.batch) + " HW=" + std::to_string(c.H) + "x" +
               std::to_string(c.W) + " cfg=" + route.config;
    }
    if (note) detail += (detail.empty() ? "" : " ") + std::string(note);
    pending.push_back({name, flops, bytes >= 0.0 ? bytes : (shape ? conv_algo_bytes(*shape) : 0.0), a, b, detail});
    return route;
  }

  void collect() {
    const char* log_path = getenv("DDMI_LAUNCH_LOG");
    FILE* log = log_path ? fopen(log_path, "a") : nullptr;
    for (auto& p : pending) {
      DD_HIP_CHECK(hipEventSynchronize(p.b));
      float ms = 0;
      DD_HIP_CHECK(hipEventElapsedTime(&ms, p.a, p.b));
      KStat& s = stats[p.name];
      s.ms += ms;
      s.n += 1;
      s.flops += p.flops;
      s.bytes += p.bytes;
      if (log) fprintf(log, "%s\t%s\t%.6g\t%.6f\t%.6g\n", p.name.c_str(), p.detail.c_str(), p.flops, ms, p.bytes);
      ev_pool.push_back(p.a);
      ev_pool.push_back(p.b);
    }
    pending.clear();
    if (log) fclose(log);
  }

  ConvArgs attach(ConvArgs a, size_t w, size_t b, const SplitW& x) {
    a.wgt = W(w);
    a.bias = W(b);
    if (gemm_mode == DD_GEMM_FP32 || x.hi == kNone) return a;
    a.prec = gemm_mode == DD_GEMM_BF16 ? 1 : 0;
    a.wh = reinterpret_cast<const uint16_t*>(W(a.prec ? x.b16 : x.hi));
    a.wl = reinterpret_cast<const uint16_t*>(W(x.lo));
    a.wsinv = W(x.sinv);
    a.ldh = x.ldh;
    a.flags = num_flags;
    return a;
  }
  ConvRoute run(ConvArgs a, double fl, bool splitk = false, const char* note = nullptr) {
    const int64_t mo = (int64_t)a.Nimg * a.Ho * a.Wo * a.Cout;
    if (splitk && a.wh && a.prec == 0 && mo <= (int64_t(1) << 20)) {
      a.split_cap = 8 * mo;
      a.split_part = buf(in_side ? "x3_split_side" : "x3_split_main", (size_t)a.split_cap);
    }
    return launch(a.wh ? "conv_x3" : "conv_gemm", fl, [&] { return launch_conv_gemm(a, st); }, &a, -1.0, note);
  }

  struct PoolSpec {
    View4 out, add;
    int oh = 0, ow = 0;
  };

  static ConvGeom geom(const Conv& c) { return {c.k, c.k, c.stride, c.pad, c.cout}; }
  ConvRoute conv(const Conv& c, View4 in, int N, int H, int Wd, View4 out, bool relu, View4 res = {},
                 const PoolSpec* pool = nullptr) {
    ConvArgs a = attach(conv_args(in, N, H, Wd, c.cin, geom(c), out, relu, res), c.w, c.b, c.x3);
    if (pool && a.Ho % pool->oh == 0 && a.Wo % pool->ow == 0 && a.Ho / pool->oh == a.Wo / pool->ow)
      pool_into(a, a.Ho / pool->oh, pool->out, pool->add);
    return run(a, 2.0 * N * a.Ho * a.Wo * (double)c.cout * c.k * c.k * c.cin_real, true);
  }
  ConvRoute conv_c(const Conv& c, const float* in, int N, int H, int Wd, float* out, bool relu,
                   const float* res = nullptr, const PoolSpec* pool = nullptr) {
    const int Ho = (H + 2 * c.pad - c.k) / c.stride + 1, Wo = (Wd + 2 * c.pad - c.k) / c.stride + 1;
    return conv(c, nhwc(in, H, Wd, c.cin), N, H, Wd, nhwc(out, Ho, Wo, c.cout), relu, nhwc(res, Ho, Wo, c.cout), pool);
  }
  void stem_and_pool(const Conv& c, const float* in4, int N, int H, int Wd, float* stem, float* pool, int hp, int wp,
                     int in_idx, int in_c, int in_u8 = 0, const float* lut = nullptr) {
    const int hs = (H + 2 * c.pad - c.k) / c.stride + 1, ws = (Wd + 2 * c.pad - c.k) / c.stride + 1;
    const ConvArgs a = attach(
        conv_args(nhwc(in4, H, Wd, c.cin), N, H, Wd, c.cin, geom(c), nhwc(stem, hs, ws, c.cout), true), c.w, c.b, c.x3);
    const double fl = 2.0 * N * hs * ws * (double)c.cout * c.k * c.k * c.cin_real;
    const bool nchw = use_nchw_stem();
    const double in_bytes = nchw ? (double)N * H * Wd * in_c * (in_u8 ? 1.0 : 4.0) : (double)N * H * Wd * c.cin * 4.0;
    const double wb = (a.wh && a.prec == 1) ? 2.0 : 4.0;
    const double bytes = in_bytes + 4.0 * N * hp * wp * c.cout + wb * (double)c.cout * c.k * c.k * c.cin;
    const ConvRoute r = launch("stem_pool", fl, [&] {
      return launch_stem_pool(a, pool, hp, wp, st, nchw ? in_tab + in_idx : nullptr, nchw ? in_c : 0,
                              nchw ? in_u8 : 0, lut);
    }, nullptr, bytes);
    if (r.kernel) return;
    if (nchw) throw std::runtime_error("stem: the NCHW-input fused stem refused this shape (DDMI_STEM_NCHW=0 avoids it)");
    conv_c(c, in4, N, H, Wd, stem, true);
    launch("pool", 0, [&] { launch_maxpool3x3s2(stem, pool, N, hs, ws, c.cout, hp, wp, st); });
  }

  void gemm_g(const Lin& L, View4 A, int G, int R, View4 C, bool relu = false, View4 res = {}, int64_t route_rows = 0) {
    ConvArgs a = attach(gemm_args(A, G, R, L.nin, L.nout, C, relu, res), L.w, L.b, L.x3);
    a.route_rows = route_rows;
    run(a, 2.0 * G * R * (double)L.nout * L.nin);
  }
  static View4 dense(const float* p, int M, int64_t ld) { return row_view(p, (int64_t)M * ld, ld); }
  void gemm(const Lin& L, const float* A, int M, float* C, bool relu = false, const float* res = nullptr) {
    gemm_g(L, dense(A, M, L.nin), 1, M, dense(C, M, L.nout), relu, res ? dense(res, M, L.nout) : View4{});
  }
  bool gemm_ln(const Lin& L, const float* A, int M, float* C, const float* res, const LNp& p, float* Y) {
    ConvArgs a = attach(gemm_args(dense(A, M, L.nin), 1, M, L.nin, L.nout, dense(C, M, L.nout), false,
                                  dense(res, M, L.nout)), L.w, L.b, L.x3);
    if (ln_fold && p.c == L.nout) fold_ln(a, Y, W(p.g), W(p.b));
    return run(a, 2.0 * M * (double)L.nout * L.nin).ln;
  }
  void gemm_slice(const Lin& L, int k0, int kn, bool with_bias, View4 A, int G, int R, View4 C, bool relu,
                  View4 res = {}) {
    if (k0 % 8 || kn % 8 || k0 + kn > L.nin) throw std::runtime_error("gemm_slice: bad K slice");
    ConvArgs a = attach(gemm_args(A, G, R, kn, L.nout, C, relu, res), L.w, with_bias ? L.b : kNone, L.x3);
    slice_k(a, k0, L.nin);
    run(a, 2.0 * G * R * (double)L.nout * kn);
  }

  void ln(const LNp& p, const float* x, int64_t ldx, float* y, int64_t ldy, int rows, const float* res = nullptr,
          int64_t ldres = 0, int res_div = 1, const float* fs = nullptr, const float* fb = nullptr, int film_div = 0,
          int64_t film_ld = 0) {
    launch("layernorm", 0, [&] {
      launch_layernorm(x, ldx, res, ldres, res_div, W(p.g), W(p.b), fs, fb, y, ldy, rows, p.c, st, film_div, film_ld);
    });
  }
  void ln_g(const LNp& p, const float* x, float* y, int64_t ld, int G, int R, int64_t gs) {
    launch("layernorm", 0, [&] {
      launch_layernorm(x, ld, nullptr, 0, 1, W(p.g), W(p.b), nullptr, nullptr, y, ld, G * R, p.c, st, 0, 0, R, gs);
    });
  }

  float* run_stage(const TrunkW& t, int s, const float* x, int B, int& H, int& Wd, const std::string& tag,
                   const PoolSpec* pool = nullptr, bool* pooled = nullptr) {
    if (pooled) *pooled = false;
    const std::vector<Block>& blocks = t.stages[s];
    const int stride = s == 0 ? 1 : 2;
    const int Ho = (H + 2 - 3) / stride + 1, Wo = (Wd + 2 - 3) / stride + 1;
    const int outc = t.ch[1 + s];
    const size_t n_out = (size_t)B * Ho * Wo * outc;
    const int mid = blocks[0].bottleneck ? outc / 4 : outc;
    float* bufA = buf(tag + "_s" + std::to_string(s) + "_a", n_out);
    float* bufB = buf(tag + "_s" + std::to_string(s) + "_b", n_out);
    float* tmp1 = buf(tag + "_s" + std::to_string(s) + "_t1", (size_t)B * std::max(H * Wd, Ho * Wo) * mid);
    float* tmp2 = buf(tag + "_s" + std::to_string(s) + "_t2", (size_t)B * Ho * Wo * mid);
    float* dsb = buf(tag + "_s" + std::to_string(s) + "_ds", n_out);
    bool all_pooled = true;
    const float* cur = x;
    int ch = H, cw = Wd;
    {
      const int nb = B;
      float* outs[2] = {bufA, bufB};
      for (size_t b = 0; b < blocks.size(); ++b) {
        const Block& blk = blocks[b];
        float* y = outs[b & 1];
        const float* sc = cur;
        const int bs = b == 0 ? stride : 1;
        const int oh = (ch + 2 - 3) / bs + 1, ow = (cw + 2 - 3) / bs + 1;
        if (blk.has_ds) {
          conv_c(blk.ds, cur, nb, ch, cw, dsb, false);
          sc = dsb;
        }
        const PoolSpec* bp = b + 1 == blocks.size() ? pool : nullptr;
        ConvRoute r;
        if (!blk.bottleneck) {
          conv_c(blk.c1, cur, nb, ch, cw, tmp2, true);
          r = conv_c(blk.c2, tmp2, nb, oh, ow, y, true, sc, bp);
        } else {
          conv_c(blk.c1, cur, nb, ch, cw, tmp1, true);
          conv_c(blk.c2, tmp1, nb, ch, cw, tmp2, true);
          r = conv_c(blk.c3, tmp2, nb, oh, ow, y, true, sc, bp);
        }
        if (bp) all_pooled = r.pooled;
        cur = y;
        ch = oh;
        cw = ow;
      }
    }
    if (pool && pooled) *pooled = all_pooled;
    H = ch;
    Wd = cw;
    return ((blocks.size() - 1) & 1) ? bufB : bufA;
  }

  PoolSpec img_pool_spec(int i, int B) {
    const int C = gpt[i].C, T = 320;
    return {hwc(buf("gpt_x", (size_t)B * T * C), (int64_t)T * C, 32, C), hwc(W(gpt[i].pos), 0, 32, C), 8, 32};
  }
  PoolSpec lid_pool_spec(int i, int B) {
    const int Cl = lid.ch[1 + i];
    return {nhwc(buf("gpt_lpool", (size_t)B * 64 * Cl), 8, 8, Cl), View4{}, 8, 8};
  }
  void fuse(int i, float* imgf, int B, int Hi, int Wi, float* lidf, int Hl, int Wl, bool img_pooled = false,
            bool lid_pooled = false) {
    const GptW& g = gpt[i];
    const int C = g.C, Cl = lid.ch[1 + i];
    const int T = 320, nimg = 256;
    const int hs = C / 4;
    float* X = buf("gpt_x", (size_t)B * T * C);
    float* Hb = buf("gpt_h", (size_t)B * T * C);
    float* QKV = buf("gpt_qkv", (size_t)B * T * 3 * C);
    float* Y = buf("gpt_y", (size_t)B * T * C);
    float* MLP = buf("gpt_mlp", (size_t)B * T * 4 * C);
    float* LP = buf("gpt_lpool", (size_t)B * 64 * Cl);
    float* LO = buf("gpt_lout", (size_t)B * 64 * Cl);
    const View4 xo = hwc(X, (int64_t)T * C, 32, C), lpo = nhwc(LP, 8, 8, Cl);
    if (!img_pooled) launch("pool", 0, [&] { launch_avgpool(imgf, B, Hi, Wi, C, 8, 32, xo, W(g.pos), st); });
    if (!lid_pooled) launch("pool", 0, [&] { launch_avgpool(lidf, B, Hl, Wl, Cl, 8, 8, lpo, nullptr, st); });
    conv(l2i[i], lpo, B, 8, 8, hwc(X + (size_t)nimg * C, (int64_t)T * C, 8, C), false,
         hwc(W(g.pos) + (size_t)nimg * C, 0, 8, C));
    const int M = B * T;
    bool hb_ready = false;
    const bool last_rows = gpt_last_rows && i + 1 == 4;
    for (size_t bi = 0; bi < g.blocks.size(); ++bi) {
      const GptBlockW& w = g.blocks[bi];
      if (!hb_ready) ln(w.ln1, X, C, Hb, C, M);
      const bool live = last_rows && bi + 1 == g.blocks.size();
      gemm(w.qkv, Hb, M, QKV);
      const int aprec = (gemm_mode == DD_GEMM_FP32 || !gpt_attn_x3 || C / 4 > 128 || T % 32 || T > 1024)
                            ? 0
                            : (gemm_mode == DD_GEMM_BF16 ? 2 : 1);
      if (live) {
        const int nl = T - nimg;
        const int64_t gs = (int64_t)T * C, off = (int64_t)nimg * C;
        launch("attn", 4.0 * B * nl * T * (double)C,
               [&] { launch_gpt_attention(QKV, B, T, C, 4, Y, aprec, st, nimg, nl); });
        const View4 xl = row_view(X + off, gs, C), hl = row_view(Hb + off, gs, C);
        gemm_g(w.proj, row_view(Y + off, gs, C), B, nl, xl, false, xl, M);
        ln_g(w.ln2, X + off, Hb + off, C, B, nl, gs);
        const View4 ml = row_view(MLP + (int64_t)nimg * 4 * C, 4 * gs, 4 * C);
        gemm_g(w.mlp0, hl, B, nl, ml, true, {}, M);
        gemm_g(w.mlp2, ml, B, nl, xl, false, xl, M);
        ln_g(g.lnf, X + off, Hb + off, C, B, nl, gs);
        hb_ready = true;
        continue;
      }
      launch("attn", 4.0 * B * T * T * (double)C, [&] { launch_gpt_attention(QKV, B, T, C, 4, Y, aprec, st); });
      const LNp& nx = bi + 1 < g.blocks.size() ? g.blocks[bi + 1].ln1 : g.lnf;
      const bool tail_on = gpt_tail_env >= 0 ? gpt_tail_env != 0 : B <= 16;
      if (tail_on && ln_fold && gemm_mode == DD_GEMM_F16X3 && gpt_tail_supported(C) && w.ln2.c == C && nx.c == C &&
          w.proj.x3.hi != kNone && w.mlp0.x3.hi != kNone && w.mlp2.x3.hi != kNone) {
        auto tw = [&](const Lin& L) {
          GptTailW t;
          t.wh = reinterpret_cast<const uint16_t*>(W(L.x3.hi));
          t.wl = reinterpret_cast<const uint16_t*>(W(L.x3.lo));
          t.sinv = W(L.x3.sinv);
          t.bias = W(L.b);
          t.ldh = L.x3.ldh;
          return t;
        };
        GptTailArgs t;
        t.y = Y;
        t.x = X;
        t.hb = Hb;
        t.M = M;
        t.C = C;
        t.proj = tw(w.proj);
        t.up = tw(w.mlp0);
        t.down = tw(w.mlp2);
        t.ln2_g = W(w.ln2.g);
        t.ln2_b = W(w.ln2.b);
        t.lnn_g = W(nx.g);
        t.lnn_b = W(nx.b);
        t.flags = num_flags;
        launch("gpt_tail", 2.0 * M * 9.0 * C * C, [&] { launch_gpt_tail(t, st); });
        hb_ready = true;
        continue;
      }
      if (!gemm_ln(w.proj, Y, M, X, X, w.ln2, Hb))
        ln(w.ln2, X, C, Hb, C, M);
      gemm(w.mlp0, Hb, M, MLP, true);
      hb_ready = gemm_ln(w.mlp2, MLP, M, X, X, nx, Hb);
    }
    if (!hb_ready) ln(g.lnf, X, C, Hb, C, M);
    const View4 gl = nhwc(LO, 8, 8, Cl);
    conv(i2l[i], hwc(Hb + (size_t)nimg * C, (int64_t)T * C, 8, C), B, 8, 8, gl, false);
    if (i + 1 < 4) {
      const View4 gi = hwc(Hb, (int64_t)T * C, 32, C), io = nhwc(imgf, Hi, Wi, C);
      launch("bilinear", 0, [&] { launch_bilinear(gi, B, 8, 32, C, io, Hi, Wi, 8.0f / Hi, 32.0f / Wi, 1, st); });
    }
    const View4 lo = nhwc(lidf, Hl, Wl, Cl);
    launch("bilinear", 0, [&] { launch_bilinear(gl, B, 8, 8, Cl, lo, Hl, Wl, 8.0f / Hl, 8.0f / Wl, 1, st); });
  }

  int head_mode() const { return gemm_mode == DD_GEMM_BF16 ? DD_GEMM_F16X3 : gemm_mode; }
  bool use_nchw_stem() const { return stem_nchw && gemm_mode != DD_GEMM_FP32 && cfg.lidar_channels <= 3; }
  struct ModeScope {
    Model* m;
    int saved;
    ModeScope(Model* mm, int mode) : m(mm), saved(mm->gemm_mode) { m->gemm_mode = mode; }
    ~ModeScope() { m->gemm_mode = saved; }
  };

  std::vector<int> denoise_timesteps(int steps) const {
    const bool vanilla = schedule == DD_SCHED_VANILLA;
    std::vector<int> roll(steps);
    const int ratio = vanilla ? 1000 / steps : 1;
    for (int s = 0; s < steps; ++s)
      roll[steps - 1 - s] = vanilla ? s * ratio
                                    : (int)std::nearbyint((double)s * ((double)cfg.step_span / (double)steps));
    return roll;
  }
  std::string film_key;
  void ensure_film(int steps) {
    const std::string k = std::to_string(steps) + "/" + std::to_string(schedule) + "/" + std::to_string(gemm_mode);
    if (k == film_key) return;
    film_key.clear();
    time_film(steps);
    film_key = k;
  }
  void time_film(int steps) {
    ModeScope head_scope(this, head_mode());
    const int d = 256;
    const std::vector<int> roll = denoise_timesteps(steps);
    float* te0 = buf("temb0", d);
    float* te1 = buf("temb1", 4 * d);
    float* te2 = buf("temb2", d);
    float* mte = buf("temb_mish", d);
    for (int si = 0; si < steps; ++si) {
      const int k = roll[si];
      launch("misc", 0, [&] { launch_timestep_embed((float)k, te0, d, st); });
      gemm(tm1, te0, 1, te1);
      launch("misc", 0, [&] { launch_activation(te1, te1, 4 * d, 0, st); });
      gemm(tm3, te1, 1, te2);
      launch("misc", 0, [&] { launch_activation(te2, mte, d, 0, st); });
      for (int l = 0; l < 2; ++l)
        gemm(dl[l].film, mte, 1, buf("film_s" + std::to_string(si) + "l" + std::to_string(l), 2 * d));
    }
  }

  void train_time_film(int B) {
    const int d = 256;
    const int* t = reinterpret_cast<const int*>(bufs.at("in_tsteps").first);
    float* te0 = buf("train_temb0", (size_t)B * d);
    float* te1 = buf("train_temb1", (size_t)B * 4 * d);
    float* te2 = buf("train_temb2", (size_t)B * d);
    float* mte = buf("train_temb_mish", (size_t)B * d);
    launch("misc", 0, [&] { launch_timestep_embed_rows(t, te0, B, d, st); });
    gemm(tm1, te0, B, te1);
    launch("misc", 0, [&] { launch_activation(te1, te1, (int64_t)B * 4 * d, 0, st); });
    gemm(tm3, te1, B, te2);
    launch("misc", 0, [&] { launch_activation(te2, mte, (int64_t)B * d, 0, st); });
    for (int l = 0; l < 2; ++l) gemm(dl[l].film, mte, B, buf("train_film_l" + std::to_string(l), (size_t)B * 2 * d));
    float* sa = buf("train_sa", B);
    float* s1a = buf("train_s1a", B);
    launch("misc", 0, [&] { launch_train_coeffs(t, ac_dev, sa, s1a, B, 1000, st); });
  }

  void train_loss_partials(const Call& c, int B) {
    if (!c.train || !c.target) return;
    const int Q = cfg.num_modes, P = cfg.num_poses;
    for (int l = 0; l < 2; ++l) {
      const std::string sf = "_s0l" + std::to_string(l);
      float* part = buf("train_part_l" + std::to_string(l), (size_t)2 * B);
      launch("misc", 0, [&] {
        launch_traj_loss_scene(bufs.at("reg" + sf).first, bufs.at("cls" + sf).first, bufs.at("in_target").first,
                               W(anchor), part, B, Q, P, st);
      });
    }
  }

  void forward_body(const Call& c) {
    const int B = c.B, steps = c.steps;
    const bool heads = c.heads();
    const int d = 256, Q = cfg.num_modes, P = cfg.num_poses;
    const int HC = cfg.cam_h, WC = cfg.cam_w, HL = cfg.lidar_h, WL = cfg.lidar_w;
    const bool nchw = use_nchw_stem();
    float* cam4 = nchw ? nullptr : bufs.at("in_cam4").first;
    float* lid4 = nchw ? nullptr : bufs.at("in_lid4").first;
    const float* stat = bufs["in_status"].first;
// ... 1207 lines not shown
```

diffusiondrive_amd/csrc/weights.cpp:

```cpp
#include "weights.h"

#include <algorithm>
#include <cmath>
#include <cstdint>
#include <cstring>

namespace ddmi {

BlobIndex::BlobIndex(const void* blob, size_t bytes) {
  const uint8_t* p = static_cast<const uint8_t*>(blob);
  const uint8_t* end = p + bytes;
  auto need = [&](size_t n) {
    if (p > end || (size_t)(end - p) < n) throw std::invalid_argument("weight blob truncated");
  };
  auto align16 = [&]() {
    const size_t off = ((size_t)(p - static_cast<const uint8_t*>(blob)) + 15) & ~size_t(15);
    if (off > bytes) throw std::invalid_argument("weight blob truncated");
    p = static_cast<const uint8_t*>(blob) + off;
  };
  need(8);
  if (std::memcmp(p, "DDW1", 4) != 0) throw std::invalid_argument("weight blob: bad magic (expected DDW1)");
  uint32_t count;
  std::memcpy(&count, p + 4, 4);
  p += 8;
  for (uint32_t i = 0; i < count; ++i) {
    need(4);
    uint32_t nl;
    std::memcpy(&nl, p, 4);
    p += 4;
    need(nl);
    std::string name(reinterpret_cast<const char*>(p), nl);
    p += nl;
    need(4);
    uint32_t nd;
    std::memcpy(&nd, p, 4);
    p += 4;
    if (nd > 8) throw std::invalid_argument("weight blob: ndim > 8 for " + name);
    HostTensor t;
    need(8 * (size_t)nd);
    size_t numel = 1;
    for (uint32_t d = 0; d < nd; ++d) {
      int64_t v;
      std::memcpy(&v, p, 8);
      p += 8;
      if (v < 0) throw std::invalid_argument("weight blob: negative dim for " + name);
      if (v > 0 && numel > (SIZE_MAX / 4) / (size_t)v) throw std::invalid_argument("weight blob: tensor too large: " + name);
      t.shape.push_back(v);
      numel *= (size_t)v;
    }
    need(4);
    uint32_t dtype;
    std::memcpy(&dtype, p, 4);
    p += 4;
    if (dtype != 0) throw std::invalid_argument("weight blob: unsupported dtype for " + name);
    align16();
    need(numel * 4);
    t.data = reinterpret_cast<const float*>(p);
    t.numel = numel;
    p += numel * 4;
    align16();
    map_[name] = t;
  }
}

const HostTensor& BlobIndex::get(const std::string& name, std::initializer_list<int64_t> shape) const {
  auto it = map_.find(name);
  if (it == map_.end()) throw std::invalid_argument("missing weight: " + name);
  const HostTensor& t = it->second;
  std::vector<int64_t> want(shape);
  if (t.shape != want) {
    std::string s = "shape mismatch for " + name + ": got (";
    for (auto v : t.shape) s += std::to_string(v) + ",";
    s += ") expected (";
    for (auto v : want) s += std::to_string(v) + ",";
    throw std::invalid_argument(s + ")");
  }
  return t;
}

bool BlobIndex::has(const std::string& name) const { return map_.count(name) != 0; }

size_t Arena::add(const float* data, size_t n) {
  size_t off = host_.size();
  host_.insert(host_.end(), data, data + n);
  host_.resize((host_.size() + 15) & ~size_t(15), 0.f);
  return off;
}

size_t Arena::add(const std::vector<float>& v) { return add(v.data(), v.size()); }

size_t Arena::add_zero(size_t n) {
  size_t off = host_.size();
  host_.resize(off + n, 0.f);
  host_.resize((host_.size() + 15) & ~size_t(15), 0.f);
  return off;
}

SplitW prep_split(Arena& ar, const float* w, int rows, int K) {
  SplitW x;
  x.ldh = (K + 7) / 8 * 8;
  const size_t nh = (size_t)rows * x.ldh;
  x.hi = ar.add_zero((nh + 1) / 2);
  x.lo = ar.add_zero((nh + 1) / 2);
  x.b16 = ar.add_zero((nh + 1) / 2);
  std::vector<float> sinv(rows, 1.f);
  _Float16* hi = reinterpret_cast<_Float16*>(ar.host(x.hi));
  _Float16* lo = reinterpret_cast<_Float16*>(ar.host(x.lo));
  __bf16* b16 = reinterpret_cast<__bf16*>(ar.host(x.b16));
  for (int r = 0; r < rows; ++r) {
    float amax = 0.f;
    for (int k = 0; k < K; ++k) amax = std::max(amax, std::fabs(w[(size_t)r * K + k]));
    int e = 0;
    if (amax > 0.f && std::isfinite(amax)) {
      int ex;
      std::frexp(amax, &ex);
      e = 15 - ex;
      e = std::min(e, kSplitMaxExp);
    }
    const float s = std::ldexp(1.0f, e);
    sinv[r] = std::ldexp(1.0f, -e);
    for (int k = 0; k < K; ++k) {
      const float v = w[(size_t)r * K + k] * s;
      const _Float16 h = (_Float16)v;
      hi[(size_t)r * x.ldh + k] = h;
      lo[(size_t)r * x.ldh + k] = (_Float16)(v - (float)h);
      b16[(size_t)r * x.ldh + k] = (__bf16)v;
    }
  }
  x.sinv = ar.add(sinv);
  return x;
}

void Arena::upload() {
  if (dev_) DD_HIP_CHECK(hipFree(dev_));
  DD_HIP_CHECK(hipMalloc(&dev_, std::max<size_t>(host_.size(), 16) * sizeof(float)));
  DD_HIP_CHECK(hipMemcpy(dev_, host_.data(), host_.size() * sizeof(float), hipMemcpyHostToDevice));
}

Arena::~Arena() {
  if (dev_) (void)hipFree(dev_);
}

Conv prep_conv(const BlobIndex& bx, Arena& ar, const std::string& wname, int cout, int cin, int k, int stride,
               int pad, const std::string& bn_prefix, const std::string& bias_name) {
  const HostTensor& w = bx.get(wname, {cout, cin, k, k});
  const int cin_p = (cin + 3) / 4 * 4;
  std::vector<double> scale(cout, 1.0), shift(cout, 0.0);
  if (!bn_prefix.empty()) {
    const HostTensor& g = bx.get(bn_prefix + ".weight", {cout});
    const HostTensor& b = bx.get(bn_prefix + ".bias", {cout});
    const HostTensor& m = bx.get(bn_prefix + ".running_mean", {cout});
    const HostTensor& v = bx.get(bn_prefix + ".running_var", {cout});
    for (int o = 0; o < cout; ++o) {
      const double s = (double)g.data[o] / std::sqrt((double)v.data[o] + 1e-5);
      scale[o] = s;
      shift[o] = (double)b.data[o] - (double)m.data[o] * s;
    }
  }
  if (!bias_name.empty()) {
    const HostTensor& b = bx.get(bias_name, {cout});
    for (int o = 0; o < cout; ++o) shift[o] += (double)b.data[o];
  }
  std::vector<float> wl((size_t)cout * k * k * cin_p, 0.f);
  for (int o = 0; o < cout; ++o)
    for (int i = 0; i < cin; ++i)
      for (int y = 0; y < k; ++y)
        for (int x = 0; x < k; ++x)
          wl[(((size_t)o * k + y) * k + x) * cin_p + i] =
              (float)((double)w.data[(((size_t)o * cin + i) * k + y) * k + x] * scale[o]);
  std::vector<float> bl(cout);
  bool any_bias = !bn_prefix.empty() || !bias_name.empty();
  for (int o = 0; o < cout; ++o) bl[o] = (float)shift[o];
  Conv c;
  c.x3 = prep_split(ar, wl.data(), cout, k * k * cin_p);
  c.w = ar.add(wl);
  c.b = any_bias ? ar.add(bl) : kNone;
  c.cout = cout;
  c.cin = cin_p;
  c.cin_real = cin;
  c.k = k;
  c.stride = stride;
  c.pad = pad;
  return c;
}

Lin prep_linear(const BlobIndex& bx, Arena& ar, const std::string& prefix, int nout, int nin, bool bias) {
  const HostTensor& w = bx.get(prefix + ".weight", {nout, nin});
  Lin l;
  l.w = ar.add(w.data, w.numel);
  l.x3 = prep_split(ar, w.data, nout, nin);
  l.b = bias ? ar.add(bx.get(prefix + ".bias", {nout}).data, (size_t)nout) : kNone;
  l.nout = nout;
  l.nin = nin;
  return l;
}

Lin prep_linear_rows(const BlobIndex& bx, Arena& ar, const std::string& wname, const std::string& bname, int rows_total,
                     int nin, int row0, int nrows) {
  const HostTensor& w = bx.get(wname, {rows_total, nin});
  const HostTensor& b = bx.get(bname, {rows_total});
  Lin l;
  l.w = ar.add(w.data + (size_t)row0 * nin, (size_t)nrows * nin);
  l.x3 = prep_split(ar, w.data + (size_t)row0 * nin, nrows, nin);
  l.b = ar.add(b.data + row0, (size_t)nrows);
  l.nout = nrows;
  l.nin = nin;
  return l;
}

LNp prep_ln(const BlobIndex& bx, Arena& ar, const std::string& prefix, int c) {
  LNp l;
  l.g = ar.add(bx.get(prefix + ".weight", {c}).data, (size_t)c);
  l.b = ar.add(bx.get(prefix + ".bias", {c}).data, (size_t)c);
  l.c = c;
  return l;
}

}
```

diffusiondrive_amd/csrc/weights.h:

```cpp
#pragma once
#include <initializer_list>
#include <string>
#include <unordered_map>
#include <vector>

#include "common.h"

namespace ddmi {

constexpr size_t kNone = ~size_t(0);

struct HostTensor {
  std::vector<int64_t> shape;
  const float* data = nullptr;
  size_t numel = 0;
};

class BlobIndex {
 public:
  BlobIndex(const void* blob, size_t bytes);
  const HostTensor& get(const std::string& name, std::initializer_list<int64_t> shape) const;
  bool has(const std::string& name) const;

 private:
  std::unordered_map<std::string, HostTensor> map_;
};

class Arena {
 public:
  size_t add(const float* data, size_t n);
  size_t add(const std::vector<float>& v);
  size_t add_zero(size_t n);
  float* host(size_t off) { return host_.data() + off; }
  void upload();
  const float* ptr(size_t off) const { return off == kNone ? nullptr : dev_ + off; }
  size_t bytes() const { return host_.size() * sizeof(float); }
  ~Arena();

 private:
  std::vector<float> host_;
  float* dev_ = nullptr;
};

struct SplitW {
  size_t hi = kNone, lo = kNone, sinv = kNone;
  size_t b16 = kNone;
  int ldh = 0;
};
struct Conv {
  size_t w = kNone, b = kNone;
  int cout = 0, cin = 0, cin_real = 0, k = 1, stride = 1, pad = 0;
  SplitW x3;
};
struct Lin {
  size_t w = kNone, b = kNone;
  int nout = 0, nin = 0;
  SplitW x3;
};
struct LNp {
  size_t g = kNone, b = kNone;
  int c = 0;
};

Conv prep_conv(const BlobIndex& bx, Arena& ar, const std::string& wname, int cout, int cin, int k, int stride,
               int pad, const std::string& bn_prefix, const std::string& bias_name);
Lin prep_linear(const BlobIndex& bx, Arena& ar, const std::string& prefix, int nout, int nin, bool bias = true);
Lin prep_linear_rows(const BlobIndex& bx, Arena& ar, const std::string& wname, const std::string& bname,
                     int rows_total, int nin, int row0, int nrows);
SplitW prep_split(Arena& ar, const float* w, int rows, int K);

LNp prep_ln(const BlobIndex& bx, Arena& ar, const std::string& prefix, int c);

}
```

include/ddmi.h:

```cpp
#ifndef DDMI_H_
#define DDMI_H_

#include <stddef.h>
#include <stdint.h>

#ifdef __cplusplus
extern "C" {
#endif

#define DD_ABI_VERSION 1

#define DD_OK 0
#define DD_ERR_INVALID -1
#define DD_ERR_RUNTIME -2

typedef struct dd_handle dd_handle;

#define DD_MAX_MODES 128

typedef struct dd_config {
  int abi_version;
  int image_arch;
  int lidar_arch;
  int cam_h, cam_w;
  int lidar_h, lidar_w;
  int lidar_channels;
  int num_modes;
  int num_poses;
  int trunc_timestep;
  int step_span;
} dd_config;

typedef struct dd_outputs {
  float* trajectory;
  float* poses_reg;
  float* poses_cls;
  float* bev_semantic_map;
  float* agent_states;
  float* agent_labels;
} dd_outputs;

#define DD_MAX_SAMPLES 32
typedef struct dd_sample_outputs {
  float* trajectory;
  float* poses_reg;
  float* poses_cls;
  float* best_trajectory;
  int*   best_index;
  float* bev_semantic_map;
  float* agent_states;
  float* agent_labels;
} dd_sample_outputs;

typedef struct dd_train_outputs {
  float* trajectory;
  float* poses_reg[2];
  float* poses_cls[2];
  float* loss;
  float* bev_semantic_map;
  float* agent_states;
  float* agent_labels;
} dd_train_outputs;

typedef struct dd_inputs {
  const float* camera_f32;
  const uint8_t* camera_u8;
  const float* lidar_f32;
  const uint8_t* lidar_u8;
  int lidar_hist_max;
  const float* status;
  const float* noise;
} dd_inputs;

void dd_default_config(dd_config* cfg);

int dd_create(const dd_config* cfg, const void* weights_blob, size_t blob_bytes, int device, dd_handle** out);

int dd_forward(dd_handle* h, const float* camera, const float* lidar, const float* status, const float* noise,
               int B, int steps, float* out_traj, float* out_modes, float* out_cls, void* stream);

int dd_forward_ex(dd_handle* h, const float* camera, const float* lidar, const float* status, const float* noise,
                  int B, int steps, const dd_outputs* outs, void* stream);

int dd_forward_in(dd_handle* h, const dd_inputs* in, int B, int steps, const dd_outputs* outs, void* stream);

int dd_forward_samples(dd_handle* h, const float* camera, const float* lidar, const float* status,
                       const float* noise , int B, int S, int steps,
                       const dd_sample_outputs* outs, void* stream);

int dd_forward_samples_in(dd_handle* h, const dd_inputs* in, int B, int S, int steps, const dd_sample_outputs* outs,
                          void* stream);

int dd_forward_train(dd_handle* h, const float* camera, const float* lidar, const float* status, const float* noise,
                     const int* timesteps, const float* target_traj, int B, float cls_weight, float reg_weight,
                     const dd_train_outputs* outs, void* stream);
int dd_forward_train_in(dd_handle* h, const dd_inputs* in, const int* timesteps, const float* target_traj, int B,
                        float cls_weight, float reg_weight, const dd_train_outputs* outs, void* stream);
int dd_bev_semantic_loss(const float* logits, const unsigned char* target, int B, int C, int H, int W, float* work,
                         float* loss, void* stream);
size_t dd_bev_semantic_loss_work(int B, int H, int W);

int dd_destroy(dd_handle* h);

int dd_set_seed(dd_handle* h, unsigned long long seed);
int dd_set_seed_at(dd_handle* h, unsigned long long seed, unsigned long long first_scene);

const char* dd_last_error(void);

int dd_set_profiling(dd_handle* h, int enable);
int dd_reset_stats(dd_handle* h);
int dd_kernel_stats(dd_handle* h, const char* kernel, double* total_ms, long long* launches, double* flops);
int dd_kernel_bytes(dd_handle* h, const char* kernel, double* bytes);
int dd_set_graph(dd_handle* h, int enable);
int dd_set_streams(dd_handle* h, int n);
int dd_get_streams(dd_handle* h, int* n);
int dd_graph_info(dd_handle* h, int* programs, int* segments, int* multi_stream_execs);
int dd_graph_nodes(dd_handle* h, int* kernel_nodes, int* other_nodes);
#define DD_GEMM_FP32 0
#define DD_GEMM_F16X3 1
#define DD_GEMM_BF16 2
int dd_set_gemm_mode(dd_handle* h, int mode);
int dd_get_gemm_mode(dd_handle* h, int* mode);
#define DD_SCHED_TRUNCATED 0
#define DD_SCHED_VANILLA 1
int dd_set_schedule(dd_handle* h, int schedule);
#define DD_NUM_F16_OVERFLOW_BIT 1u
#define DD_NUM_SYNC_TIMEOUT_BIT 2u
#define DD_NUM_SYNC_STATE_BIT 4u
int dd_numerics_flags(dd_handle* h, unsigned* flags, int clear);
int dd_tap(dd_handle* h, const char* name, float* dst, size_t count, size_t* actual, void* stream);

typedef struct dd_sim_params {
  double wheel_base;
  double dt;
  int tracking_horizon;
  double q_lon, r_lon;
  double q_lat[3], r_lat;
  double jerk_penalty;
  double curvature_rate_penalty;
  double initial_curvature_penalty;
  double stopping_gain;
  double stopping_velocity;
  double max_steering_angle;
  double accel_time_constant;
  double steering_time_constant;
} dd_sim_params;
void dd_default_sim_params(dd_sim_params* p);
size_t dd_simulate_work(int N);
int dd_simulate_proposals(const double* proposals, const double* ego_states, int N, int per_group,
                          const dd_sim_params* params, double* work, double* out_states, void* stream);
int dd_simulate(const float* traj, int num_poses, const double* ego_states, int N, int per_group,
                const dd_sim_params* params, double* work, double* out_states, void* stream);

typedef struct dd_comfort_params {
  double dt;
  double min_lon_accel;
  double max_lon_accel;
  double max_abs_lat_accel;
  double max_abs_mag_jerk;
  double max_abs_lon_jerk;
  double max_abs_yaw_accel;
  double max_abs_yaw_rate;
} dd_comfort_params;
void dd_default_comfort_params(dd_comfort_params* p);
int dd_comfort(const double* states, int N, const dd_comfort_params* params, uint8_t* out_flags, double* out_signals,
               void* stream);

typedef struct dd_area_params {
  double half_length;
  double half_width;
  double rear_axle_to_center;
  double dt;
  double driving_direction_horizon;
  double driving_direction_compliance_threshold;
  double driving_direction_violation_threshold;
} dd_area_params;
void dd_default_area_params(dd_area_params* p);
typedef struct dd_drivable_maps {
  const double* verts;
  const int32_t* ring_off;
  const int32_t* poly_ring_off;
  const uint8_t* poly_kind;
  const int32_t* scene_poly_off;
  int num_polys;
} dd_drivable_maps;
size_t dd_ego_areas_work(int P);
int dd_ego_areas(const double* states, int N, int per_group, const dd_drivable_maps* maps, int G,
                 const dd_area_params* params, double* work, uint8_t* out_areas, double* out_scores,
                 double* out_progress, double* out_coords, void* stream);

int dd_build_camera(const uint8_t* cams, int B, int src_h, int src_w, float* out, int out_h, int out_w,
                    void* stream);
int dd_build_lidar(const float* xyz, const int64_t* offsets, int B, int channels, float* out, int resolution,
                   float range_lo, float range_hi, int pixels_per_meter, float max_height, float split_height,
                   int hist_max, long long max_points, void* stream);

int dd_build_camera_u8(const uint8_t* cams, int B, int src_h, int src_w, uint8_t* out, int out_h, int out_w,
                       void* stream);
int dd_build_lidar_u8(const float* xyz, const int64_t* offsets, int B, int channels, uint8_t* out, int resolution,
                      float range_lo, float range_hi, int pixels_per_meter, float max_height, float split_height,
                      int hist_max, long long max_points, void* stream);

const char* dd_op_last_error(void);
const char* dd_op_last_kernel(void);
int dd_op_split_weights(const float* w, int rows, int K, uint16_t* hi, uint16_t* lo, uint16_t* b16, float* sinv,
                        int* ldh_out);
int dd_op_pack_mk_weights(const float* w, int nout, int nin, uint16_t* packed, float* sinv);
int dd_op_mk_linear(const float* A, int K, const float* wgt, const float* bias, float* out, int N, void* stream);
int dd_op_bevproj(const float* p3, int64_t p3_ld, const float* kvp, const float* wgt, const float* bias,
                  const float* ln_g, const float* ln_b, float* out, int B, int H, int W, int Hk, int Wk, void* stream);
int dd_op_conv2d(const float* in, int B, int H, int W, int Cin, const float* wgt, const float* bias,
                 const float* res, float* out, int Cout, int KH, int KW, int stride, int pad, int relu, void* stream);
int dd_op_conv2d_x3(const float* in, int B, int H, int W, int Cin, const float* wgt, const float* bias,
                    const float* res, float* out, int Cout, int KH, int KW, int stride, int pad, int relu, int prec,
                    unsigned* flags, void* stream);
int dd_op_stem_pool_x3(const float* in, int B, int H, int W, const float* wgt, const float* bias, float* out,
                       unsigned* flags, void* stream);
int dd_op_stem_pool(const float* in, int B, int H, int W, const float* wgt, const float* bias, float* out, int prec,
                    unsigned* flags, void* stream);
int dd_op_stem_pool_nchw(const float* in, int B, int C, int H, int W, const float* wgt, const float* bias, float* out,
                         int prec, unsigned* flags, void* stream);
int dd_op_stem_pool_u8(const uint8_t* in, int layout, int B, int C, int H, int W, const float* lut, const float* wgt,
                       const float* bias, float* out, int prec, unsigned* flags, void* stream);
int dd_op_gemm(const float* A, int M, int K, const float* W, const float* bias, const float* res, float* C, int N,
               int relu, void* stream);
int dd_op_gemm_batched(const float* A, const float* Bm, float* C, int batch, int M, int N, int K, int kn,
                       void* stream);
int dd_op_layernorm(const float* x, const float* res, int res_div, const float* g, const float* b,
                    const float* film_scale, const float* film_shift, float* y, int rows, int C, void* stream);
int dd_op_softmax_rows(float* x, int rows, int L, float scale, void* stream);
int dd_op_bilinear(const float* in, int B, int Hi, int Wi, int C, float* out, int Ho, int Wo, void* stream);
int dd_op_bilinear_add(const float* in, int B, int Hi, int Wi, int C, float* out, int Ho, int Wo, void* stream);
int dd_op_maxpool3x3s2(const float* in, int B, int H, int W, int C, float* out, void* stream);
int dd_op_avgpool(const float* in, int B, int H, int W, int C, int oh, int ow, float* out, void* stream);
int dd_op_bev_sample_attn(const float* logits, const float* pts, const float* value, float* out, int B, int Q,
                          int P, int Hv, int Wv, int C, void* stream);
int dd_op_mha_small(const float* q, const float* k, const float* v, float* out, int B, int Lq, int Lk, int nh,
                    int hd, void* stream);
int dd_op_gpt_attention(const float* qkv, float* y, int B, int T, int C, int heads, int prec, void* stream);
int dd_op_gpt_attention_rows(const float* qkv, float* y, int B, int T, int C, int heads, int prec, int q_first,
                             int q_count, int waves, void* stream);
int dd_op_layernorm_groups(const float* x, const float* g, const float* b, float* y, int groups, int group_rows,
                           long long group_stride, int C, void* stream);

typedef struct dd_op_view {
  float* p;
  int64_t sn, sh, sw, sc;
} dd_op_view;
typedef struct dd_op_conv_desc {
  dd_op_view in, out, res;
  int N, H, W, Cin;
  int KH, KW, stride, pad, Cout;
  const float* wgt;
  int64_t ldb;
  int k0;
  const float* bias;
  int relu;
  int mode;
  unsigned* flags;
  int64_t route_rows;
  float* ln_out;
  const float* ln_g;
  const float* ln_b;
  dd_op_view pool_out;
  int pool_p;
  dd_op_view pool_add;
  int fused_ln;
  int fused_pool;
} dd_op_conv_desc;
size_t dd_op_conv_desc_size(void);
int dd_op_conv_view(dd_op_conv_desc* d, void* stream);
int dd_op_layernorm_ld(const float* x, int64_t ldx, const float* res, int64_t ldres, int res_div, const float* g,
                       const float* b, const float* film_scale, const float* film_shift, int film_div,
                       int64_t film_ld, float* y, int64_t ldy, int rows, int C, void* stream);
int dd_op_bilinear_view(const dd_op_view* in, int B, int Hi, int Wi, int C, const dd_op_view* out, int Ho, int Wo,
                        int accumulate, void* stream);

#ifdef __cplusplus
}
#endif
#endif
```

Before: 5705.

## Add Winograd F(2,3) row-transform path to the x6 3x3 conv kernel

Result: faster. 5987 (median of 6 runs) (+4.9%).

```diff
diff --git a/diffusiondrive_amd/_lib.py b/diffusiondrive_amd/_lib.py
--- a/diffusiondrive_amd/_lib.py
+++ b/diffusiondrive_amd/_lib.py
@@ -170,6 +170,7 @@
                               ctypes.POINTER(ctypes.c_size_t), c_void_p]),
     "dd_op_last_error": (ctypes.c_char_p, []),
     "dd_op_last_kernel": (ctypes.c_char_p, []),
+    "dd_op_last_walk": (ctypes.c_char_p, []),
     "dd_op_split_weights": (ctypes.c_int, [c_void_p, ctypes.c_int, ctypes.c_int, c_void_p, c_void_p, c_void_p, c_void_p,
                                            ctypes.POINTER(ctypes.c_int)]),
     "dd_op_pack_mk_weights": (ctypes.c_int, [c_void_p, ctypes.c_int, ctypes.c_int, c_void_p, c_void_p]),
diff --git a/diffusiondrive_amd/csrc/common.h b/diffusiondrive_amd/csrc/common.h
--- a/diffusiondrive_amd/csrc/common.h
+++ b/diffusiondrive_amd/csrc/common.h
@@ -70,6 +70,10 @@
   int64_t ldh = 0;
   unsigned* flags = nullptr;
   int prec = 0;
+  const uint16_t* wh2 = nullptr;
+  const uint16_t* wl2 = nullptr;
+  const float* wsinv2 = nullptr;
+  int64_t ldh2 = 0;
   const int* rowmap = nullptr;
   int rowmap_nimg = 0;
   int rowmap_groups = 0;
@@ -309,6 +313,7 @@
 struct ConvRoute {
   const char* kernel = nullptr;
   const char* config = "";
+  const char* walk = "";
   bool pooled = false;
   bool ln = false;
 };
diff --git a/diffusiondrive_amd/csrc/conv_x6.hip b/diffusiondrive_amd/csrc/conv_x6.hip
--- a/diffusiondrive_amd/csrc/conv_x6.hip
+++ b/diffusiondrive_amd/csrc/conv_x6.hip
@@ -74,11 +74,11 @@
   return make_uint2(__builtin_bit_cast(uint32_t, b01), __builtin_bit_cast(uint32_t, b23));
 }
 
-constexpr bool halo_in_window(int t, int D, int TA, bool first) {
+constexpr bool halo_in_window(int t, int D, int TA, bool first, int S = 9) {
   for (int j = 1; j <= D; ++j) {
     const int u = t - j;
     if (first && u < 0) return false;
-    if (((u % 9) + 9) % 9 == TA) return true;
+    if (((u % S) + S) % S == TA) return true;
   }
   return false;
 }
@@ -98,17 +98,23 @@
 #define X6_STAMP(k)
 #endif
 
-template <int TH, int TW, int BN, int WM, int WN, int D, int NSLOT, int SH, int PREC>
+template <int TH, int TW, int BN, int WM, int WN, int D, int NSLOT, int SH, int PREC, int WALK = 0>
 __global__ __launch_bounds__(64 * WM * WN, SH >= 2 ? SH + 1 : (SH ? (WM * WN == 8 ? 4 : 2) : 1)) void conv_x6_kernel(ConvArgs a, int tiles_x, int tiles_y, int n_sp,
                                                                int ntn, int nchunks) {
   constexpr int NW = WM * WN, NT = 64 * NW;
   constexpr int BM = TH * TW;
-  constexpr int TM = BM / WM / 32;
+  constexpr int MR = WALK ? BM / 2 : BM;
+  constexpr int NPL = WALK ? 4 : 1;
+  constexpr int NSTEP = WALK ? 12 : 9;
+  constexpr int PW = TW / 2;
+  constexpr int TM = MR / WM / 32;
   constexpr int TN = BN / WN / 32;
-  static_assert(TM >= 1 && TN >= 1 && TM * WM * 32 == BM && TN * WN * 32 == BN, "wave tiling");
+  static_assert(TM >= 1 && TN >= 1 && TM * WM * 32 == MR && TN * WN * 32 == BN, "wave tiling");
   static_assert(NSLOT >= D + 1 && D >= 1 && D <= 8, "ring");
+  static_assert(!WALK || (PREC == 0 && SH == 0 && NW == 8 && TM == 1 && (PW == 8 || PW == 16)), "walk forms");
+  constexpr bool ONEBUF = SH || WALK;
   constexpr int P = TW + 2;
-  constexpr int HP = (TH + 2) * P;
+  constexpr int HP = WALK ? (TH + 2) * PW * 4 : (TH + 2) * P;
   constexpr int ABYTES = HP * 128;
   constexpr int BIMG = BN * 64;
   constexpr int BSLOT = 2 * BIMG;
@@ -117,9 +123,10 @@
   static_assert(BPS >= 1 && (2 * BQ) % NW == 0 && BQ % BPS == 0, "B DMA split over the waves");
   constexpr int CH = PREC ? 64 : 32;
   constexpr int QP = CH / 4;
-  constexpr int ALD = (HP * QP + NT - 1) / NT;
+  constexpr int AE = ((TH + 2) * PW * QP + NT - 1) / NT;
+  constexpr int ALD = WALK ? 4 * AE : (HP * QP + NT - 1) / NT;
   constexpr int TA = 1;
-  constexpr int NHB = SH ? 1 : 2;
+  constexpr int NHB = ONEBUF ? 1 : 2;
   constexpr int B_OFF = NHB * ABYTES;
   constexpr int LDS_MAIN = NHB * ABYTES + NSLOT * BSLOT, LDS_EPI = BM * BN * 4;
   __shared__ __attribute__((aligned(1024))) char lds[LDS_MAIN > LDS_EPI ? LDS_MAIN : LDS_EPI];
@@ -151,7 +158,7 @@
 
   const x6i4 rin = rsrc6(a.in);
 
-  constexpr bool HKEEP = NW == 8 && ALD <= 12 && !SH;
+  constexpr bool HKEEP = NW == 8 && ALD <= 12 && !SH && !WALK;
   auto hofs_of = [&](int i) {
     const int e = tid + NT * i;
     const int px = e / QP, q = e % QP;
@@ -175,10 +182,31 @@
       hwad[i] = hwad_of(i);
     }
   }
+  auto opaque_tid = [&]() {
+    int t = tid;
+    asm volatile("" : "+v"(t));
+    return t;
+  };
   x6f4 hr[ALD];
   auto halo_issue = [&](int c) {
     const bool cv = c < nchunks;
     const int co = c * CH;
+    if constexpr (WALK) {
+      const int tq = opaque_tid();
+#pragma unroll
+      for (int i = 0; i < AE; ++i) {
+        const int pr = (tq + NT * i) >> 3, q = tq & 7;
+        const int hy = pr / PW, p = pr - hy * PW;
+        const int iy = oy0 - 1 + hy, ix0 = ox0 - 1 + 2 * p;
+        const bool rv = cv && hy < TH + 2 && (unsigned)iy < (unsigned)a.H;
+        const int ho = (int)(nimg * a.in_sn + iy * a.in_sh + ix0 * a.in_sw) + 4 * q + co;
+#pragma unroll
+        for (int k = 0; k < 4; ++k)
+          hr[4 * i + k] = vload6(rin, (rv && (unsigned)(ix0 + k) < (unsigned)a.W)
+                                          ? (uint32_t)(ho + k * (int)a.in_sw) * 4u : kOOB6);
+      }
+      return;
+    }
 #pragma unroll
     for (int i = 0; i < ALD; ++i) {
       const int ho = HKEEP ? hofs[HKEEP ? i : 0] : hofs_of(i);
@@ -191,6 +219,27 @@
   };
   auto halo_store = [&](int buf) {
     char* base = lds + buf * ABYTES;
+    if constexpr (WALK) {
+      const int tq = opaque_tid();
+#pragma unroll
+      for (int i = 0; i < AE; ++i) {
+        const int pr = (tq + NT * i) >> 3, q = tq & 7;
+        const int hy = pr / PW, p = pr - hy * PW;
+        if (hy >= TH + 2) continue;
+        const int swz = PW == 8 ? ((p >> 1) & 3) | ((hy & 1) << 2) : (p >> 1) & 7;
+        const int hw = (hy * 4 * PW + p) * 128 + ((((q >> 1) ^ swz) & 7) << 4) + ((q & 1) << 3);
+        const x6f4 d0 = hr[4 * i], d1 = hr[4 * i + 1], d2 = hr[4 * i + 2], d3 = hr[4 * i + 3];
+        const x6f4 v[4] = {d0 - d2, d1 + d2, d2 - d1, d1 - d3};
+#pragma unroll
+        for (int xi = 0; xi < 4; ++xi) {
+          uint2 hi, lo;
+          split4(v[xi], hi, lo);
+          *reinterpret_cast<uint2*>(base + xi * PW * 128 + hw) = hi;
+          *reinterpret_cast<uint2*>(base + xi * PW * 128 + (hw ^ 64)) = lo;
+        }
+      }
+      return;
+    }
 #pragma unroll
     for (int i = 0; i < ALD; ++i) {
       const int hw = HKEEP ? hwad[HKEEP ? i : 0] : hwad_of(i);
@@ -217,15 +266,17 @@
     const int ls = (lane & 3) ^ ((c >> 2) & 3);
     const int n = n0 + c;
     bok[j] = n < a.Cout;
-    boff[j] = (uint32_t)(n * (int)a.ldh + ls * 8) * 2u;
+    boff[j] = (uint32_t)(n * (int)(WALK ? a.ldh2 : a.ldh) + ls * 8) * 2u;
     brow[j] = rb;
   }
   const bool bimg_lo = (wave * BPS) / BQ == 1;
-  const x6i4 rwb = rsrc6((bimg_lo && !PREC) ? (const void*)a.wl : (const void*)a.wh);
+  const x6i4 rwb = WALK ? rsrc6(bimg_lo ? (const void*)a.wl2 : (const void*)a.wh2)
+                        : rsrc6((bimg_lo && !PREC) ? (const void*)a.wl : (const void*)a.wh);
   const uint32_t kb_lo = (PREC && bimg_lo) ? 64u : 0u;
   auto b_issue = [&](int slot, int tap, int c) {
     const bool cv = c < nchunks;
-    const uint32_t kb = (uint32_t)(tap * Cin + c * CH) * 2u + kb_lo;
+    const uint32_t kbv = (uint32_t)(tap * Cin + c * CH) * 2u + kb_lo;
+    const uint32_t kb = WALK ? (uint32_t)__builtin_amdgcn_readfirstlane((int)kbv) : kbv;
 #pragma unroll
     for (int j = 0; j < BPS; ++j) {
       const uint32_t dst = lds_u32 + B_OFF + slot * BSLOT + (bimg_lo ? BIMG : 0) + brow[j] * 64;
@@ -239,6 +290,12 @@
 #pragma unroll
   for (int i = 0; i < TM; ++i) {
     const int m = (wm * TM + i) * 32 + li;
+    if constexpr (WALK) {
+      const int y = m / PW, p = m % PW;
+      const int swz = PW == 8 ? ((p >> 1) & 3) | ((y & 1) << 2) : (p >> 1) & 7;
+      aad[i][0] = aad[i][1] = aad[i][2] = (y * 4 * PW + p) * 128 + (((hh ^ swz) & 7) << 4);
+      continue;
+    }
     const int y = m / TW, x = m % TW;
 #pragma unroll
     for (int kw = 0; kw < 3; ++kw) aad[i][kw] = (y * P + x + kw) * 128 + (((hh ^ ((x + kw) >> 1)) & 7) << 4);
@@ -250,9 +307,9 @@
     bad_[j] = c * 64 + (((hh ^ (c >> 2)) & 3) << 4);
   }
 
-  x6f16 acc[TM][TN];
-#pragma unroll
-  for (int i = 0; i < TM; ++i)
+  x6f16 acc[NPL * TM][TN];
+#pragma unroll
+  for (int i = 0; i < NPL * TM; ++i)
 #pragma unroll
     for (int j = 0; j < TN; ++j)
 #pragma unroll
@@ -265,8 +322,10 @@
   Frag F0, F1;
   auto load_frag = [&](Frag& F, int slot, int c, auto TAP, auto S2) {
     constexpr int t = decltype(TAP)::value, s2 = decltype(S2)::value;
-    constexpr int kh = t / 3, kw = t % 3;
-    const char* abuf = lds + (SH ? 0 : (c & 1)) * ABYTES + kh * P * 128;
+    constexpr int kh = WALK ? t / 4 : t / 3, kw = WALK ? 0 : t % 3;
+    constexpr int aofs = WALK ? (kh * 4 + t % 4) * PW * 128 : kh * P * 128;
+    constexpr int axor = (WALK && PW == 8 && (kh & 1)) ? 64 : 0;
+    const char* abuf = lds + (ONEBUF ? 0 : (c & 1)) * ABYTES + aofs;
     const char* bbuf = lds + B_OFF + slot * BSLOT;
 #pragma unroll
     for (int j = 0; j < TN; ++j) {
@@ -276,54 +335,55 @@
     }
 #pragma unroll
     for (int i = 0; i < TM; ++i) {
-      const int o = aad[i][kw] ^ (32 * s2);
+      const int o = aad[i][kw] ^ (32 * s2) ^ axor;
       F.ah[i] = *reinterpret_cast<const x6h8*>(abuf + o);
       F.al[i] = *reinterpret_cast<const x6h8*>(abuf + (o ^ 64));
     }
   };
-  auto mfma_frag = [&](const Frag& F) {
+  auto mfma_frag = [&](const Frag& F, auto TAP) {
+    constexpr int pl = WALK ? decltype(TAP)::value % 4 : 0;
     if constexpr (PREC == 1) {
 #pragma unroll
       for (int i = 0; i < TM; ++i)
 #pragma unroll
         for (int j = 0; j < TN; ++j)
-          acc[i][j] = __builtin_amdgcn_mfma_f32_32x32x16_bf16(__builtin_bit_cast(x6b8, F.ah[i]),
-                                                             __builtin_bit_cast(x6b8, F.bh[j]), acc[i][j], 0, 0, 0);
+          acc[pl * TM + i][j] = __builtin_amdgcn_mfma_f32_32x32x16_bf16(__builtin_bit_cast(x6b8, F.ah[i]),
+                                                             __builtin_bit_cast(x6b8, F.bh[j]), acc[pl * TM + i][j], 0, 0, 0);
 #pragma unroll
       for (int i = 0; i < TM; ++i)
 #pragma unroll
         for (int j = 0; j < TN; ++j)
-          acc[i][j] = __builtin_amdgcn_mfma_f32_32x32x16_bf16(__builtin_bit_cast(x6b8, F.al[i]),
-                                                             __builtin_bit_cast(x6b8, F.bl[j]), acc[i][j], 0, 0, 0);
+          acc[pl * TM + i][j] = __builtin_amdgcn_mfma_f32_32x32x16_bf16(__builtin_bit_cast(x6b8, F.al[i]),
+                                                             __builtin_bit_cast(x6b8, F.bl[j]), acc[pl * TM + i][j], 0, 0, 0);
       return;
     }
 #pragma unroll
     for (int i = 0; i < TM; ++i)
 #pragma unroll
       for (int j = 0; j < TN; ++j)
-        acc[i][j] = __builtin_amdgcn_mfma_f32_32x32x16_f16(F.al[i], F.bh[j], acc[i][j], 0, 0, 0);
+        acc[pl * TM + i][j] = __builtin_amdgcn_mfma_f32_32x32x16_f16(F.al[i], F.bh[j], acc[pl * TM + i][j], 0, 0, 0);
 #pragma unroll
     for (int i = 0; i < TM; ++i)
 #pragma unroll
       for (int j = 0; j < TN; ++j)
-        acc[i][j] = __builtin_amdgcn_mfma_f32_32x32x16_f16(F.ah[i], F.bl[j], acc[i][j], 0, 0, 0);
+        acc[pl * TM + i][j] = __builtin_amdgcn_mfma_f32_32x32x16_f16(F.ah[i], F.bl[j], acc[pl * TM + i][j], 0, 0, 0);
 #pragma unroll
     for (int i = 0; i < TM; ++i)
 #pragma unroll
       for (int j = 0; j < TN; ++j)
-        acc[i][j] = __builtin_amdgcn_mfma_f32_32x32x16_f16(F.ah[i], F.bh[j], acc[i][j], 0, 0, 0);
+        acc[pl * TM + i][j] = __builtin_amdgcn_mfma_f32_32x32x16_f16(F.ah[i], F.bh[j], acc[pl * TM + i][j], 0, 0, 0);
   };
 
   int slot = 0;
   auto open_step = [&](int c, auto TAP, auto FIRST) {
     constexpr int t = decltype(TAP)::value;
     constexpr bool first = decltype(FIRST)::value;
-    constexpr int N = (D - 1) * BPS + (halo_in_window(t, D, TA, first) ? ALD : 0);
+    constexpr int N = (D - 1) * BPS + (halo_in_window(t, D, TA, first, NSTEP) ? ALD : 0);
     step_barrier<N>();
-    constexpr int tn = (t + D) % 9;
+    constexpr int tn = (t + D) % NSTEP;
     int ns = slot + D;
     if (ns >= NSLOT) ns -= NSLOT;
-    b_issue(ns, tn, t + D >= 9 ? c + 1 : c);
+    b_issue(ns, tn, t + D >= NSTEP ? c + 1 : c);
     if constexpr (t == TA) halo_issue(c + 1);
   };
 
@@ -339,45 +399,47 @@
   auto step = [&](int c, auto TAP, auto FIRST) {
     constexpr int t = decltype(TAP)::value;
     constexpr bool first = decltype(FIRST)::value;
+    constexpr int TL = NSTEP - 1;
     if constexpr (!PIPE) {
       load_frag(F0, slot, c, TAP, std::integral_constant<int, 0>());
-      mfma_frag(F0);
+      mfma_frag(F0, TAP);
       load_frag(F0, slot, c, TAP, std::integral_constant<int, 1>());
-      mfma_frag(F0);
-      if constexpr (t == 8) {
-        wait_vm<(8 - TA) * BPS>();
+      mfma_frag(F0, TAP);
+      if constexpr (t == TL) {
+        wait_vm<(TL - TA) * BPS>();
         halo_tie();
         asm volatile("s_waitcnt lgkmcnt(0)\n\ts_barrier" ::: "memory");
         halo_store(0);
       }
       if (++slot == NSLOT) slot = 0;
-      open_step(t == 8 ? c + 1 : c, std::integral_constant<int, (t + 1) % 9>(),
-                std::integral_constant<bool, first && t != 8>());
+      open_step(t == TL ? c + 1 : c, std::integral_constant<int, (t + 1) % NSTEP>(),
+                std::integral_constant<bool, first && t != TL>());
       return;
     }
     load_frag(F1, slot, c, TAP, std::integral_constant<int, 1>());
     __builtin_amdgcn_sched_barrier(0);
-    mfma_frag(F0);
-    if constexpr (t == 8) {
-      wait_vm<(8 - TA) * BPS>();
+    mfma_frag(F0, TAP);
+    if constexpr (t == TL) {
+      wait_vm<(TL - TA) * BPS>();
       halo_tie();
-      if constexpr (SH) {
+      if constexpr (ONEBUF) {
         asm volatile("s_waitcnt lgkmcnt(0)\n\ts_barrier" ::: "memory");
         halo_store(0);
       } else {
         halo_store((c + 1) & 1);
       }
     }
-    constexpr int t1 = (t + 1) % 9;
-    const int c1 = t == 8 ? c + 1 : c;
+    constexpr int t1 = (t + 1) % NSTEP;
+    const int c1 = t == TL ? c + 1 : c;
     if (++slot == NSLOT) slot = 0;
-    open_step(c1, std::integral_constant<int, t1>(), std::integral_constant<bool, first && t != 8>());
+    open_step(c1, std::integral_constant<int, t1>(), std::integral_constant<bool, first && t != TL>());
     load_frag(F0, slot, c1, std::integral_constant<int, t1>(), std::integral_constant<int, 0>());
     __builtin_amdgcn_sched_barrier(0);
-    mfma_frag(F1);
+    mfma_frag(F1, TAP);
     __builtin_amdgcn_sched_barrier(0);
   };
   auto chunk = [&](int c, auto FIRST) {
+    if constexpr (WALK) asm volatile("" : "+s"(slot));
     step(c, std::integral_constant<int, 0>(), FIRST);
     step(c, std::integral_constant<int, 1>(), FIRST);
     step(c, std::integral_constant<int, 2>(), FIRST);
@@ -387,6 +449,11 @@
     step(c, std::integral_constant<int, 6>(), FIRST);
     step(c, std::integral_constant<int, 7>(), FIRST);
     step(c, std::integral_constant<int, 8>(), FIRST);
+    if constexpr (WALK) {
+      step(c, std::integral_constant<int, 9>(), FIRST);
+      step(c, std::integral_constant<int, 10>(), FIRST);
+      step(c, std::integral_constant<int, 11>(), FIRST);
+    }
   };
   X6_STAMP(1);
   chunk(0, std::true_type());
@@ -404,7 +471,7 @@
   const int osh = (int)a.out_sh, osw = (int)a.out_sw;
   const int rsh = (int)a.res_sh, rsw = (int)a.res_sw;
   constexpr int IT = BM / (NT / QN);
-  constexpr bool EARLY = IT <= (NW == 8 && !SH ? 16 : 8);
+  constexpr bool EARLY = IT <= (NW == 8 && !SH ? 16 : 8) && !WALK;
   x6f4 rv[IT];
   int ooff[IT];
   auto load_res = [&]() {
@@ -420,22 +487,36 @@
   if constexpr (EARLY) load_res();
   x6f4 scl = {0.f, 0.f, 0.f, 0.f}, bia = {0.f, 0.f, 0.f, 0.f};
   if (nv) {
-    scl = *reinterpret_cast<const x6f4*>(a.wsinv + nq) * a.alpha;
+    scl = *reinterpret_cast<const x6f4*>((WALK ? a.wsinv2 : a.wsinv) + nq) * a.alpha;
     if (a.bias) bia = *reinterpret_cast<const x6f4*>(a.bias + nq);
   }
   float* ct = reinterpret_cast<float*>(lds);
-#pragma unroll
-  for (int i = 0; i < TM; ++i)
+  bool bad = false;
+  if constexpr (WALK) {
 #pragma unroll
     for (int j = 0; j < TN; ++j)
 #pragma unroll
       for (int r = 0; r < 16; ++r) {
-        const int m = (wm * TM + i) * 32 + (r & 3) + 8 * (r >> 2) + 4 * hh;
-        ct[m * BN + (wn * TN + j) * 32 + li] = acc[i][j][r];
+        const int m = wm * 32 + (r & 3) + 8 * (r >> 2) + 4 * hh;
+        const float m0 = acc[0][j][r], m1 = acc[1][j][r], m2 = acc[2][j][r], m3 = acc[3][j][r];
+        const float ev = m0 + m1 + m2, od = m1 - m2 - m3;
+        bad |= !(__builtin_isfinite(ev) && __builtin_isfinite(od));
+        ct[(2 * m) * BN + (wn * TN + j) * 32 + li] = ev;
+        ct[(2 * m + 1) * BN + (wn * TN + j) * 32 + li] = od;
       }
+  } else {
+#pragma unroll
+    for (int i = 0; i < TM; ++i)
+#pragma unroll
+      for (int j = 0; j < TN; ++j)
+#pragma unroll
+        for (int r = 0; r < 16; ++r) {
+          const int m = (wm * TM + i) * 32 + (r & 3) + 8 * (r >> 2) + 4 * hh;
+          ct[m * BN + (wn * TN + j) * 32 + li] = acc[i][j][r];
+        }
+  }
   __syncthreads();
   if constexpr (!EARLY) load_res();
-  bool bad = false;
 #pragma unroll
   for (int k = 0; k < IT; ++k) {
     if (ooff[k] < 0) continue;
@@ -481,7 +562,7 @@
 #endif
 }
 
-template <int TH, int TW, int BN, int WM, int WN, int D, int NSLOT, int SH, int PREC>
+template <int TH, int TW, int BN, int WM, int WN, int D, int NSLOT, int SH, int PREC, int WALK = 0>
 static void launch_x6_one(const ConvArgs& a_in, hipStream_t st, ConvRoute& r) {
   ConvArgs a = a_in;
   auto al16 = [](const void* p) { return (reinterpret_cast<uintptr_t>(p) & 15) == 0; };
@@ -498,7 +579,8 @@
                                   std::to_string(BN) + "," + std::to_string(WM) + "," + std::to_string(WN) +
                                   (PREC ? ",bf16>" : ">");
   r.config = name.c_str();
-  hipLaunchKernelGGL((conv_x6_kernel<TH, TW, BN, WM, WN, D, NSLOT, SH, PREC>), dim3(n_sp * ntn), dim3(64 * WM * WN), 0,
+  r.walk = WALK ? "f23" : "";
+  hipLaunchKernelGGL((conv_x6_kernel<TH, TW, BN, WM, WN, D, NSLOT, SH, PREC, WALK>), dim3(n_sp * ntn), dim3(64 * WM * WN), 0,
                      st, a, tiles_x, tiles_y, n_sp, ntn, a.Cin / (PREC ? 64 : 32));
   DD_HIP_CHECK(hipGetLastError());
 }
@@ -513,6 +595,14 @@
     if (a.prec == 1) throw std::runtime_error("conv_x6: bf16 takes the 8-wave configurations");
   }
   launch_x6_one<TH, TW, BN, WM, WN, D, NSLOT, SH, 0>(a, st, r);
+}
+
+static bool x6_walk_routed(const ConvArgs& a) {
+  static const int kShapes[][4] = {
+      {32, 128, 128, 128}, {16, 64, 256, 256}, {8, 32, 512, 512}, {32, 32, 128, 128}};
+  for (const auto& s : kShapes)
+    if (a.H == s[0] && a.W == s[1] && a.Cin == s[2] && a.Cout == s[3]) return true;
+  return false;
 }
 
 bool launch_conv_x6(const ConvArgs& a, hipStream_t st, ConvRoute& r) {
@@ -539,28 +629,46 @@
   const bool sh4 = a.prec == 0 && a.Cin <= 64;
   const bool b128 = bn128;
 #define X6(TH, TW, BN, WM, WN, D, NS, SH) launch_x6_cfg<TH, TW, BN, WM, WN, D, NS, SH>(a, st, r)
+#define X6W(TH, TW, BN, WM, WN, D, NS) launch_x6_one<TH, TW, BN, WM, WN, D, NS, 0, 0, 1>(a, st, r)
+  const char* we = getenv("DDMI_X6_WALK");
+  const int wk = we ? atoi(we) : 1;
+  const bool wimg = a.prec == 0 && a.wh2 && a.wl2 && a.wsinv2 && al16(a.wsinv2) && a.ldh2 == 12 * (int64_t)a.Cin &&
+                    (int64_t)a.Cout * a.ldh2 < (int64_t(1) << 30);
+  const bool wany = wk == 2 && wimg;
+  auto walk_by_cout = [&]() {
+    if (wide) X6W(8, 32, 128, 4, 2, 3, 4);
+    else if (a.Cout > 64) X6W(16, 16, 128, 4, 2, 3, 4);
+    else X6W(16, 16, 64, 4, 2, 2, 3);
+  };
+  const bool wr = wany || (wk == 1 && wimg && x6_walk_routed(a));
   {
     const int64_t wgs = b128 ? n_sp * ((a.Cout + 127) / 128) : n_sp * ((a.Cout + 63) / 64);
     const char* se = getenv("DDMI_X6_SMALL");
     const int sm = se ? atoi(se) : 1;
     if (sm == 2 || (wgs < 128 && sm != 0)) {
-      X6(8, 8, 64, 2, 2, 2, 3, 0);
+      if (wany && (!wide || a.Cout > 64)) walk_by_cout(); else X6(8, 8, 64, 2, 2, 2, 3, 0);
       return true;
     }
   }
   if (wide) {
     if (b128) {
-      X6(8, 32, 128, 4, 2, 3, 4, 0);
+      if (wr) X6W(8, 32, 128, 4, 2, 3, 4); else X6(8, 32, 128, 4, 2, 3, 4, 0);
     } else {
-      if (sh4) X6(8, 32, 64, 4, 1, 2, 3, 1); else X6(8, 32, 64, 4, 2, 2, 3, 0);
+      if (wany && a.Cout > 64) walk_by_cout();
+      else if (sh4) X6(8, 32, 64, 4, 1, 2, 3, 1);
+      else X6(8, 32, 64, 4, 2, 2, 3, 0);
     }
   } else {
     if (b128) {
-      X6(16, 16, 128, 4, 2, 3, 4, 0);
+      if (wr) X6W(16, 16, 128, 4, 2, 3, 4); else X6(16, 16, 128, 4, 2, 3, 4, 0);
     } else {
-      if (sh4) X6(16, 16, 64, 4, 1, 2, 3, 1); else X6(16, 16, 64, 4, 2, 2, 3, 0);
-    }
-  }
+      if (sh4 && wany) walk_by_cout();
+      else if (sh4) X6(16, 16, 64, 4, 1, 2, 3, 1);
+      else if (wany) X6W(16, 16, 64, 4, 2, 2, 3);
+      else X6(16, 16, 64, 4, 2, 2, 3, 0);
+    }
+  }
+#undef X6W
 #undef X6
   return true;
 }
diff --git a/diffusiondrive_amd/csrc/ops_abi.cpp b/diffusiondrive_amd/csrc/ops_abi.cpp
--- a/diffusiondrive_amd/csrc/ops_abi.cpp
+++ b/diffusiondrive_amd/csrc/ops_abi.cpp
@@ -11,7 +11,9 @@
 namespace {
 thread_local std::string g_op_err;
 thread_local const char* g_op_kernel = "";
+thread_local const char* g_op_walk = "";
 void ran(const ddmi::ConvRoute& r) {
+  if (*r.config) g_op_walk = r.walk;
   if (*r.config) g_op_kernel = r.config;
 }
 
@@ -38,6 +40,8 @@
 const char* dd_op_last_error(void) { return g_op_err.c_str(); }
 
 const char* dd_op_last_kernel(void) { return g_op_kernel; }
+
+const char* dd_op_last_walk(void) { return g_op_walk; }
 
 int dd_op_split_weights(const float* w, int rows, int K, uint16_t* hi, uint16_t* lo, uint16_t* b16, float* sinv,
                         int* ldh_out) {
@@ -140,6 +144,16 @@
   a.flags = flags;
 }
 
+static bool walk_geom(int KH, int KW, int stride, int pad, int Cin) {
+  return KH == 3 && KW == 3 && stride == 1 && pad == 1 && Cin % 32 == 0;
+}
+static void attach_walk(ConvArgs& a, const Arena& ar, const SplitW& xw) {
+  a.wh2 = reinterpret_cast<const uint16_t*>(ar.ptr(xw.hi));
+  a.wl2 = reinterpret_cast<const uint16_t*>(ar.ptr(xw.lo));
+  a.wsinv2 = ar.ptr(xw.sinv);
+  a.ldh2 = xw.ldh;
+}
+
 int dd_op_conv2d(const float* in, int B, int H, int W, int Cin, const float* wgt, const float* bias, const float* res,
                  float* out, int Cout, int KH, int KW, int stride, int pad, int relu, void* stream) {
   return op_guard([&] {
@@ -158,10 +172,14 @@
     DD_HIP_CHECK(hipMemcpy(hw.data(), wgt, hw.size() * sizeof(float), hipMemcpyDeviceToHost));
     Arena ar;
     const SplitW x = prep_split(ar, hw.data(), Cout, K);
+    const bool walk = prec == 0 && walk_geom(KH, KW, stride, pad, Cin);
+    SplitW xw;
+    if (walk) xw = prep_split_walk(ar, hw.data(), Cout, Cin);
     ar.upload();
     ConvArgs a = conv2d_args(in, B, H, W, Cin, wgt, bias, res, out, Cout, KH, KW, stride, pad, relu);
     if (prec != 0 && prec != 1) throw std::invalid_argument("prec must be 0 (f16x3) or 1 (bf16)");
     attach_split(a, ar, x, prec, flags);
+    if (walk) attach_walk(a, ar, xw);
     const int64_t mo = (int64_t)B * a.Ho * a.Wo * Cout;
     float* part = nullptr;
     if (prec == 0 && mo <= (1 << 20)) {
@@ -429,8 +447,12 @@
       std::vector<float> hw((size_t)d->Cout * d->ldb);
       DD_HIP_CHECK(hipMemcpy(hw.data(), d->wgt, hw.size() * sizeof(float), hipMemcpyDeviceToHost));
       const SplitW x = prep_split(ar, hw.data(), d->Cout, (int)d->ldb);
+      const bool walk = d->mode == 1 && !sliced && walk_geom(d->KH, d->KW, d->stride, d->pad, d->Cin);
+      SplitW xw;
+      if (walk) xw = prep_split_walk(ar, hw.data(), d->Cout, d->Cin);
       ar.upload();
       attach_split(a, ar, x, d->mode - 1, d->flags);
+      if (walk) attach_walk(a, ar, xw);
     }
     if (sliced) slice_k(a, d->k0, d->ldb);
     if (d->ln_out) fold_ln(a, d->ln_out, d->ln_g, d->ln_b);
diff --git a/diffusiondrive_amd/csrc/runtime.cpp b/diffusiondrive_amd/csrc/runtime.cpp
--- a/diffusiondrive_amd/csrc/runtime.cpp
+++ b/diffusiondrive_amd/csrc/runtime.cpp
@@ -1072,6 +1072,7 @@
                " K=" + std::to_string(c.KH * c.KW * c.Cin) + " k=" + std::to_string(c.KH) + " s=" +
                std::to_string(c.stride) + " z=" + std::to_string(c.batch) + " HW=" + std::to_string(c.H) + "x" +
                std::to_string(c.W) + " cfg=" + route.config;
+      if (route.walk[0]) detail += std::string(" walk=") + route.walk;
     }
     if (note) detail += (detail.empty() ? "" : " ") + std::string(note);
     pending.push_back({name, flops, bytes >= 0.0 ? bytes : (shape ? conv_algo_bytes(*shape) : 0.0), a, b, detail});
@@ -1098,7 +1099,7 @@
     if (log) fclose(log);
   }
 
-  ConvArgs attach(ConvArgs a, size_t w, size_t b, const SplitW& x) {
+  ConvArgs attach(ConvArgs a, size_t w, size_t b, const SplitW& x, const SplitW* xw = nullptr) {
     a.wgt = W(w);
     a.bias = W(b);
     if (gemm_mode == DD_GEMM_FP32 || x.hi == kNone) return a;
@@ -1108,6 +1109,12 @@
     a.wsinv = W(x.sinv);
     a.ldh = x.ldh;
     a.flags = num_flags;
+    if (xw && xw->hi != kNone && a.prec == 0) {
+      a.wh2 = reinterpret_cast<const uint16_t*>(W(xw->hi));
+      a.wl2 = reinterpret_cast<const uint16_t*>(W(xw->lo));
+      a.wsinv2 = W(xw->sinv);
+      a.ldh2 = xw->ldh;
+    }
     return a;
   }
   ConvRoute run(ConvArgs a, double fl, bool splitk = false, const char* note = nullptr) {
@@ -1127,7 +1134,7 @@
   static ConvGeom geom(const Conv& c) { return {c.k, c.k, c.stride, c.pad, c.cout}; }
   ConvRoute conv(const Conv& c, View4 in, int N, int H, int Wd, View4 out, bool relu, View4 res = {},
                  const PoolSpec* pool = nullptr) {
-    ConvArgs a = attach(conv_args(in, N, H, Wd, c.cin, geom(c), out, relu, res), c.w, c.b, c.x3);
+    ConvArgs a = attach(conv_args(in, N, H, Wd, c.cin, geom(c), out, relu, res), c.w, c.b, c.x3, &c.x3w);
     if (pool && a.Ho % pool->oh == 0 && a.Wo % pool->ow == 0 && a.Ho / pool->oh == a.Wo / pool->ow)
       pool_into(a, a.Ho / pool->oh, pool->out, pool->add);
     return run(a, 2.0 * N * a.Ho * a.Wo * (double)c.cout * c.k * c.k * c.cin_real, true);
diff --git a/diffusiondrive_amd/csrc/weights.cpp b/diffusiondrive_amd/csrc/weights.cpp
--- a/diffusiondrive_amd/csrc/weights.cpp
+++ b/diffusiondrive_amd/csrc/weights.cpp
@@ -96,17 +96,17 @@
   return off;
 }
 
-SplitW prep_split(Arena& ar, const float* w, int rows, int K) {
+SplitW prep_split(Arena& ar, const float* w, int rows, int K, bool bf16) {
   SplitW x;
   x.ldh = (K + 7) / 8 * 8;
   const size_t nh = (size_t)rows * x.ldh;
   x.hi = ar.add_zero((nh + 1) / 2);
   x.lo = ar.add_zero((nh + 1) / 2);
-  x.b16 = ar.add_zero((nh + 1) / 2);
+  if (bf16) x.b16 = ar.add_zero((nh + 1) / 2);
   std::vector<float> sinv(rows, 1.f);
   _Float16* hi = reinterpret_cast<_Float16*>(ar.host(x.hi));
   _Float16* lo = reinterpret_cast<_Float16*>(ar.host(x.lo));
-  __bf16* b16 = reinterpret_cast<__bf16*>(ar.host(x.b16));
+  __bf16* b16 = bf16 ? reinterpret_cast<__bf16*>(ar.host(x.b16)) : nullptr;
   for (int r = 0; r < rows; ++r) {
     float amax = 0.f;
     for (int k = 0; k < K; ++k) amax = std::max(amax, std::fabs(w[(size_t)r * K + k]));
@@ -124,11 +124,31 @@
       const _Float16 h = (_Float16)v;
       hi[(size_t)r * x.ldh + k] = h;
       lo[(size_t)r * x.ldh + k] = (_Float16)(v - (float)h);
-      b16[(size_t)r * x.ldh + k] = (__bf16)v;
+      if (b16) b16[(size_t)r * x.ldh + k] = (__bf16)v;
     }
   }
   x.sinv = ar.add(sinv);
   return x;
+}
+
+SplitW prep_split_walk(Arena& ar, const float* w, int cout, int cin) {
+  std::vector<float> u((size_t)cout * 12 * cin);
+  for (int o = 0; o < cout; ++o)
+    for (int y = 0; y < 3; ++y)
+      for (int i = 0; i < cin; ++i) {
+        const float* g = w + (((size_t)o * 3 + y) * 3) * cin + i;
+        const double g0 = g[0], g1 = g[cin], g2 = g[2 * (size_t)cin];
+        float* d = u.data() + (((size_t)o * 3 + y) * 4) * cin + i;
+        d[0] = (float)g0;
+        d[cin] = (float)((g0 + g1 + g2) / 2);
+        d[2 * (size_t)cin] = (float)((g0 - g1 + g2) / 2);
+        d[3 * (size_t)cin] = (float)g2;
+      }
+  return prep_split(ar, u.data(), cout, 12 * cin, false);
+}
+
+bool x6_walk_weight(int cout, int cin, int k, int stride, int pad) {
+  return k == 3 && stride == 1 && pad == 1 && cin == cout && (cin == 128 || cin == 256 || cin == 512);
 }
 
 void Arena::upload() {
@@ -173,6 +193,7 @@
   for (int o = 0; o < cout; ++o) bl[o] = (float)shift[o];
   Conv c;
   c.x3 = prep_split(ar, wl.data(), cout, k * k * cin_p);
+  if (x6_walk_weight(cout, cin_p, k, stride, pad)) c.x3w = prep_split_walk(ar, wl.data(), cout, cin_p);
   c.w = ar.add(wl);
   c.b = any_bias ? ar.add(bl) : kNone;
   c.cout = cout;
diff --git a/diffusiondrive_amd/csrc/weights.h b/diffusiondrive_amd/csrc/weights.h
--- a/diffusiondrive_amd/csrc/weights.h
+++ b/diffusiondrive_amd/csrc/weights.h
@@ -51,6 +51,7 @@
   size_t w = kNone, b = kNone;
   int cout = 0, cin = 0, cin_real = 0, k = 1, stride = 1, pad = 0;
   SplitW x3;
+  SplitW x3w;
 };
 struct Lin {
   size_t w = kNone, b = kNone;
@@ -67,7 +68,9 @@
 Lin prep_linear(const BlobIndex& bx, Arena& ar, const std::string& prefix, int nout, int nin, bool bias = true);
 Lin prep_linear_rows(const BlobIndex& bx, Arena& ar, const std::string& wname, const std::string& bname,
                      int rows_total, int nin, int row0, int nrows);
-SplitW prep_split(Arena& ar, const float* w, int rows, int K);
+SplitW prep_split(Arena& ar, const float* w, int rows, int K, bool bf16 = true);
+SplitW prep_split_walk(Arena& ar, const float* w, int cout, int cin);
+bool x6_walk_weight(int cout, int cin, int k, int stride, int pad);
 
 LNp prep_ln(const BlobIndex& bx, Arena& ar, const std::string& prefix, int c);
 
diff --git a/include/ddmi.h b/include/ddmi.h
--- a/include/ddmi.h
+++ b/include/ddmi.h
@@ -203,6 +203,7 @@
 
 const char* dd_op_last_error(void);
 const char* dd_op_last_kernel(void);
+const char* dd_op_last_walk(void);
 int dd_op_split_weights(const float* w, int rows, int K, uint16_t* hi, uint16_t* lo, uint16_t* b16, float* sinv,
                         int* ldh_out);
 int dd_op_pack_mk_weights(const float* w, int nout, int nin, uint16_t* packed, float* sinv);
```
